# vlaxose/jstsp19

Measured on AMD Instinct MI355X. Metric: channel-estimates/sec (batched MC) at Nt=Nr=64,K=64; NMSE vs ref, higher is better.
Workload: dtype c32 (storage and results fp32 complex; big contractions as split-f16 MFMA with fp32 accumulation, fp32-equivalent); 1 GPU; proposed_algorithm approximate Imax=100, Nt=Nr=64 Nrf=8 K=64 L=8 (N=64 M=4096 Gr=64 G2=512); Imax=100, outputs=S,Y,convergence_error, pilots=per-trial (B per trial), parallelism=trials sharded, dp1

## Files before the change

include/jstsp.h:

```cpp
#ifndef JSTSP_H
#define JSTSP_H

#include <stddef.h>
#include <stdint.h>

#ifdef __cplusplus
extern "C" {
#endif

typedef struct jstsp_ctx jstsp_ctx;
typedef struct { float re, im; } jstsp_c32;
typedef struct { double re, im; } jstsp_c64;

enum { JSTSP_HOST = 0, JSTSP_DEVICE = 1 };

enum {
    JSTSP_OK = 0,
    JSTSP_E_NULL = -1,
    JSTSP_E_SHAPE = -2,
    JSTSP_E_UNSUPPORTED = -3,
    JSTSP_E_ARG = -4,
    JSTSP_E_NOMEM = -5,
    JSTSP_E_ILLCOND = -6
};

enum { JSTSP_TYPE_APPROXIMATE = 0, JSTSP_TYPE_STD = 1 };

int  jstsp_create(int device_id, jstsp_ctx **out);
int  jstsp_destroy(jstsp_ctx *ctx);
int  jstsp_set_stream(jstsp_ctx *ctx, void *hip_stream);
int  jstsp_use_own_stream(jstsp_ctx *ctx);
int  jstsp_synchronize(jstsp_ctx *ctx);
const char *jstsp_last_error(void);
const char *jstsp_version(void);
size_t jstsp_workspace_bytes(const jstsp_ctx *ctx);




int jstsp_correlate_c32(jstsp_ctx *ctx, int N, int M, int Gr, int G2, int batch,
                        const jstsp_c32 *K, const jstsp_c32 *A, long long strideA,
                        const jstsp_c32 *B, long long strideB,
                        jstsp_c32 *out, int memspace);

int jstsp_synthesize_c32(jstsp_ctx *ctx, int N, int M, int Gr, int G2, int batch,
                         const jstsp_c32 *S, const jstsp_c32 *A, long long strideA,
                         const jstsp_c32 *B, long long strideB,
                         jstsp_c32 *out, int memspace);

int jstsp_gradient_head_c32(jstsp_ctx *ctx, int N, int Gr, int G2, int batch, const jstsp_c32 *Tc,
                            const jstsp_c32 *A, long long strideA, const jstsp_c32 *GA, long long strideG,
                            const jstsp_c32 *RV, jstsp_c32 *Res_out, jstsp_c32 *P1_out, int memspace);


int jstsp_proposed_algorithm_c32(jstsp_ctx *ctx, int N, int M, int Gr, int G2, int batch,
                                 const jstsp_c32 *subY, const float *Omega,
                                 const jstsp_c32 *A, long long strideA,
                                 const jstsp_c32 *B, long long strideB,
                                 int Imax, const double *tau_Y, const double *tau_S,
                                 const double *rho, int type, const int32_t *indx_S,
                                 jstsp_c32 *S_out, jstsp_c32 *Y_out, double *ce_out,
                                 int memspace);

typedef struct jstsp_pending jstsp_pending;
int jstsp_proposed_algorithm_begin_c32(jstsp_ctx *ctx, int N, int M, int Gr, int G2, int batch,
                                       const jstsp_c32 *subY, const float *Omega,
                                       const jstsp_c32 *A, long long strideA,
                                       const jstsp_c32 *B, long long strideB,
                                       int Imax, const double *tau_Y, const double *tau_S,
                                       const double *rho, int type, const int32_t *indx_S,
                                       jstsp_c32 *S_out, jstsp_c32 *Y_out, double *ce_out,
                                       jstsp_pending **pending);
int jstsp_proposed_algorithm_end(jstsp_ctx *ctx, jstsp_pending *pending, int *fallbacks);

int jstsp_last_fused_fallbacks(jstsp_ctx *ctx, int *count);

int jstsp_last_lanczos_mismatches(jstsp_ctx *ctx, int *count);

int jstsp_lambda_max_sequence_c32(jstsp_ctx *ctx, int n, int batch, int steps, const jstsp_c32 *G, float *lam, int memspace);

int jstsp_last_dictionary_block(jstsp_ctx *ctx, int *gt);

int jstsp_ls_c32(jstsp_ctx *ctx, int N, int M, int Gr, int G2, int batch, const jstsp_c32 *Y,
                 const jstsp_c32 *A, long long strideA, const jstsp_c32 *B, long long strideB,
                 jstsp_c32 *S_out, int memspace);

int jstsp_pinv_c32(jstsp_ctx *ctx, int rows, int cols, int batch, const jstsp_c32 *A, jstsp_c32 *P, int memspace);

int jstsp_last_conditioning(jstsp_ctx *ctx, double *rcond_min, double *ns_residual_max);

int jstsp_svt_c32(jstsp_ctx *ctx, int Mr, int Mt, int batch, const jstsp_c32 *Y,
                  const double *tau, jstsp_c32 *X, int memspace);

int jstsp_omp_c32(jstsp_ctx *ctx, int measures, int size_d, int batch,
                  const jstsp_c32 *A, long long strideA, const jstsp_c32 *v, int m,
                  jstsp_c32 *x_hat, int32_t *index_out, jstsp_c32 *target_out, int memspace);

int jstsp_omp_kron_c32(jstsp_ctx *ctx, int N, int M, int Gr, int G2, int batch,
                       const jstsp_c32 *Af, long long strideA, const jstsp_c32 *Bf,
                       long long strideB, const jstsp_c32 *y, int m,
                       jstsp_c32 *x_hat, int32_t *index_out, int memspace);

int jstsp_cosamp_c32(jstsp_ctx *ctx, int measures, int size_d, int batch,
                     const jstsp_c32 *A, long long strideA, const jstsp_c32 *u, int K, int iters, double tol,
                     jstsp_c32 *x_hat, int32_t *support_out, int32_t *iters_out, double *resid_out,
                     int32_t *status_out, int memspace);
int jstsp_cosamp_kron_c32(jstsp_ctx *ctx, int N, int M, int Gr, int G2, int batch,
                          const jstsp_c32 *Af, long long strideA, const jstsp_c32 *Bf, long long strideB,
                          const jstsp_c32 *y, int K, int iters, double tol,
                          jstsp_c32 *x_hat, int32_t *support_out, int32_t *iters_out, double *resid_out,
                          int32_t *status_out, int memspace);

int jstsp_mmv_omp_c32(jstsp_ctx *ctx, int N, int Gr, int S, int batch, const jstsp_c32 *A, long long strideA,
                      const jstsp_c32 *Y, int K, int pnorm, jstsp_c32 *Z_out, int32_t *index_out,
                      int32_t *count_out, int memspace);

int jstsp_sparse_admm_c32(jstsp_ctx *ctx, int Mr, int Mt, int Gr, int Gt, int batch,
                          const jstsp_c32 *Htrue, const jstsp_c32 *OH,
                          const jstsp_c32 *Dr, const jstsp_c32 *Dt, int Imax,
                          jstsp_c32 *S_out, double *ce_out, int memspace);

int jstsp_mc_svt_c32(jstsp_ctx *ctx, int Mr, int Mt, int batch, const jstsp_c32 *OH,
                     const float *Omega, int Imax, const double *tau, const double *rho,
                     jstsp_c32 *X_out, int memspace);

int jstsp_mc_admm_c32(jstsp_ctx *ctx, int Mr, int Mt, int batch, const jstsp_c32 *Htrue,
                      const jstsp_c32 *OH, const float *Omega, int Imax, const double *tau,
                      const double *rho, jstsp_c32 *X_out, double *ce_out, int memspace);

int jstsp_vamp_c32(jstsp_ctx *ctx, int M, int N, int batch, const jstsp_c32 *y, const jstsp_c32 *A,
                   long long strideA, double sigma, double L, int nit, jstsp_c32 *x_out, int memspace);

int jstsp_vamp_kron_c32(jstsp_ctx *ctx, int Na, int Gr, int G2, int batch, const jstsp_c32 *Y,
                        const jstsp_c32 *Af, long long strideA, const jstsp_c32 *Gb, long long strideG,
                        double sigma, double L, int nit, jstsp_c32 *X_out, int memspace);

int jstsp_sparse_sca_estim_f64(jstsp_ctx *ctx, long long n, const double *rhat, double rvar, double var0, double p1, double *xhat,
                               double *xvar, int memspace);
int jstsp_cawgn_estim_out_f64(jstsp_ctx *ctx, long long n, const double *y, const double *phat, double pvar, double wvar, double *zhat,
                              double *zvar, int memspace);

int jstsp_nmse_spectral_c32(jstsp_ctx *ctx, int R, int C, int batch, const jstsp_c32 *S,
                            const jstsp_c32 *Zbar, double *nmse, int memspace);

int jstsp_rate_c32(jstsp_ctx *ctx, int R, int C, int batch, const jstsp_c32 *S, const jstsp_c32 *Zbar,
                   double noise_var, double *rate, int memspace);

typedef struct jstsp_model {
    int Nt, Nr, L;
    int T_prop;
    int Mr, Mr_e;
    int Gr, Gt;
    int clusters, rays;
    int T_hbf;
    int shared_pilots;
    double noise_var;
    int beamformer;
    int rho_rule;
    double rho_scale;
    int pilots;
} jstsp_model;
enum { JSTSP_BF_ZC = 0, JSTSP_BF_DFT = 1, JSTSP_BF_QUANTIZED = 2, JSTSP_BF_QUANTIZED4 = 3 };
enum { JSTSP_RHO_MIN6 = 0, JSTSP_RHO_MAX = 1 };
enum { JSTSP_PILOTS_QAM4 = 0, JSTSP_PILOTS_GAUSS = 1 };
// ... 156 lines not shown
```

jstsp19_amd/_lib.py:

```python
from __future__ import annotations

import ctypes as C
import os

_HERE = os.path.dirname(os.path.abspath(__file__))
LIB_PATH = os.path.join(_HERE, "csrc", "libjstsp_mi355x.so")

HOST, DEVICE = 0, 1
TYPE_APPROXIMATE, TYPE_STD = 0, 1
BF_ZC, BF_DFT, BF_QUANTIZED, BF_QUANTIZED4 = 0, 1, 2, 3
RHO_MIN6, RHO_MAX = 0, 1
PILOTS_QAM4, PILOTS_GAUSS = 0, 1

c_void_p, c_int, c_ll, c_dp, c_ip = C.c_void_p, C.c_int, C.c_longlong, C.POINTER(C.c_double), C.POINTER(C.c_int)



class Model(C.Structure):
    _fields_ = [(n, c_int) for n in ("Nt", "Nr", "L", "T_prop", "Mr", "Mr_e", "Gr", "Gt", "clusters", "rays",
                                     "T_hbf", "shared_pilots")] + [("noise_var", C.c_double), ("beamformer", c_int),
                                                                   ("rho_rule", c_int), ("rho_scale", C.c_double),
                                                                   ("pilots", c_int)]


class Trials(C.Structure):
    _fields_ = [(n, c_void_p) for n in ("subY", "Omega", "A", "B", "Zbar", "H", "indx_S")] + \
               [(n, c_dp) for n in ("tau_Y", "tau_Z", "rho")] + \
               [(n, c_void_p) for n in ("Y_hbf", "A_hbf", "B_hbf", "gains", "u_r", "u_t", "noise", "qam_idx", "pilot_sym")]


class AseDesign(C.Structure):
    _fields_ = [("kind", c_int), ("n_cols", c_int), ("pool", c_int)]


SIGNATURES = {
    "jstsp_create": (c_int, [c_int, C.POINTER(c_void_p)]),
    "jstsp_destroy": (c_int, [c_void_p]),
    "jstsp_set_stream": (c_int, [c_void_p, c_void_p]),
    "jstsp_use_own_stream": (c_int, [c_void_p]),
    "jstsp_synchronize": (c_int, [c_void_p]),
    "jstsp_last_error": (C.c_char_p, []),
    "jstsp_version": (C.c_char_p, []),
    "jstsp_workspace_bytes": (C.c_size_t, [c_void_p]),
    "jstsp_correlate_c32": (c_int, [c_void_p, c_int, c_int, c_int, c_int, c_int, c_void_p, c_void_p, c_ll,
                                    c_void_p, c_ll, c_void_p, c_int]),
    "jstsp_synthesize_c32": (c_int, [c_void_p, c_int, c_int, c_int, c_int, c_int, c_void_p, c_void_p, c_ll,
                                     c_void_p, c_ll, c_void_p, c_int]),
    "jstsp_gradient_head_c32": (c_int, [c_void_p, c_int, c_int, c_int, c_int, c_void_p, c_void_p, c_ll, c_void_p, c_ll,
                                        c_void_p, c_void_p, c_void_p, c_int]),
    "jstsp_proposed_algorithm_c32": (c_int, [c_void_p, c_int, c_int, c_int, c_int, c_int, c_void_p, c_void_p,
                                             c_void_p, c_ll, c_void_p, c_ll, c_int, c_dp, c_dp, c_dp, c_int,
                                             c_void_p, c_void_p, c_void_p, c_void_p, c_int]),
    "jstsp_proposed_algorithm_begin_c32": (c_int, [c_void_p, c_int, c_int, c_int, c_int, c_int, c_void_p, c_void_p,
                                                   c_void_p, c_ll, c_void_p, c_ll, c_int, c_dp, c_dp, c_dp, c_int,
                                                   c_void_p, c_void_p, c_void_p, c_void_p, C.POINTER(c_void_p)]),
    "jstsp_proposed_algorithm_end": (c_int, [c_void_p, c_void_p, c_ip]),
    "jstsp_ls_c32": (c_int, [c_void_p, c_int, c_int, c_int, c_int, c_int, c_void_p, c_void_p, c_ll, c_void_p, c_ll,
                             c_void_p, c_int]),
    "jstsp_pinv_c32": (c_int, [c_void_p, c_int, c_int, c_int, c_void_p, c_void_p, c_int]),
    "jstsp_last_conditioning": (c_int, [c_void_p, c_dp, c_dp]),
    "jstsp_last_fused_fallbacks": (c_int, [c_void_p, c_ip]),
    "jstsp_last_lanczos_mismatches": (c_int, [c_void_p, c_ip]),
    "jstsp_last_dictionary_block": (c_int, [c_void_p, c_ip]),
    "jstsp_svt_c32": (c_int, [c_void_p, c_int, c_int, c_int, c_void_p, c_dp, c_void_p, c_int]),
    "jstsp_omp_c32": (c_int, [c_void_p, c_int, c_int, c_int, c_void_p, c_ll, c_void_p, c_int, c_void_p,
                              c_void_p, c_void_p, c_int]),
    "jstsp_omp_kron_c32": (c_int, [c_void_p, c_int, c_int, c_int, c_int, c_int, c_void_p, c_ll, c_void_p, c_ll,
                                   c_void_p, c_int, c_void_p, c_void_p, c_int]),
    "jstsp_cosamp_c32": (c_int, [c_void_p, c_int, c_int, c_int, c_void_p, c_ll, c_void_p, c_int, c_int, C.c_double, c_void_p,
                                 c_void_p, c_void_p, c_void_p, c_void_p, c_int]),
    "jstsp_cosamp_kron_c32": (c_int, [c_void_p, c_int, c_int, c_int, c_int, c_int, c_void_p, c_ll, c_void_p, c_ll, c_void_p,
                                      c_int, c_int, C.c_double, c_void_p, c_void_p, c_void_p, c_void_p, c_void_p, c_int]),
    "jstsp_mmv_omp_c32": (c_int, [c_void_p, c_int, c_int, c_int, c_int, c_void_p, c_ll, c_void_p, c_int, c_int, c_void_p,
                                  c_void_p, c_void_p, c_int]),
    "jstsp_rate_c32": (c_int, [c_void_p, c_int, c_int, c_int, c_void_p, c_void_p, C.c_double, c_void_p, c_int]),
    "jstsp_sparse_admm_c32": (c_int, [c_void_p, c_int, c_int, c_int, c_int, c_int, c_void_p, c_void_p,
                                      c_void_p, c_void_p, c_int, c_void_p, c_void_p, c_int]),
    "jstsp_mc_svt_c32": (c_int, [c_void_p, c_int, c_int, c_int, c_void_p, c_void_p, c_int, c_dp, c_dp,
                                 c_void_p, c_int]),
    "jstsp_mc_admm_c32": (c_int, [c_void_p, c_int, c_int, c_int, c_void_p, c_void_p, c_void_p, c_int, c_dp,
                                  c_dp, c_void_p, c_void_p, c_int]),
    "jstsp_vamp_c32": (c_int, [c_void_p, c_int, c_int, c_int, c_void_p, c_void_p, c_ll, C.c_double, C.c_double, c_int,
                               c_void_p, c_int]),
    "jstsp_vamp_kron_c32": (c_int, [c_void_p, c_int, c_int, c_int, c_int, c_void_p, c_void_p, c_ll, c_void_p, c_ll,
                                    C.c_double, C.c_double, c_int, c_void_p, c_int]),
    "jstsp_sparse_sca_estim_f64": (c_int, [c_void_p, c_ll, c_void_p, C.c_double, C.c_double, C.c_double, c_void_p, c_void_p, c_int]),
    "jstsp_cawgn_estim_out_f64": (c_int, [c_void_p, c_ll, c_void_p, c_void_p, C.c_double, C.c_double, c_void_p, c_dp, c_int]),
    "jstsp_lambda_max_sequence_c32": (c_int, [c_void_p, c_int, c_int, c_int, c_void_p, c_void_p, c_int]),
    "jstsp_nmse_spectral_c32": (c_int, [c_void_p, c_int, c_int, c_int, c_void_p, c_void_p, c_void_p, c_int]),
    "jstsp_build_trials_c32": (c_int, [c_void_p, C.POINTER(Model), C.c_uint64, c_int, c_ll, c_int, C.POINTER(Trials),
                                       c_int]),
    "jstsp_beamformer_c32": (c_int, [c_void_p, c_int, c_int, c_void_p, c_int]),
    "jstsp_ase_c32": (c_int, [c_void_p, c_int, c_int, c_int, c_int, c_int, c_void_p, c_void_p, c_void_p, C.c_double, c_void_p,
                              c_int]),
    "jstsp_ase_trials_c32": (c_int, [c_void_p, C.POINTER(Model), C.POINTER(AseDesign), c_int, C.c_uint64, c_int, c_ll, c_int,
                                     c_void_p, c_void_p, c_int]),
    "jstsp_singular_values_c32": (c_int, [c_void_p, c_int, c_int, c_int, c_void_p, c_void_p, c_int]),
    "jstsp_rank_trials_c32": (c_int, [c_void_p, C.POINTER(Model), C.c_uint64, c_int, c_ll, c_int, c_int, c_void_p, c_int]),
    "jstsp_set_profiling": (c_int, [c_void_p, c_int]),
    "jstsp_get_profile": (c_int, [c_void_p, C.c_char_p, c_ip, c_dp]),
}


for _n in ("correlate", "synthesize", "proposed_algorithm", "svt", "omp", "sparse_admm", "mc_svt", "mc_admm", "vamp", "ls", "pinv",
           "mmv_omp", "vamp_kron", "nmse_spectral", "rate", "beamformer", "ase", "singular_values", "cosamp", "cosamp_kron"):
    SIGNATURES["jstsp_%s_c64" % _n] = SIGNATURES["jstsp_%s_c32" % _n]


for _n in ("correlate", "synthesize", "proposed_algorithm", "svt"):
    SIGNATURES["jstsp_%s_f64" % _n] = SIGNATURES["jstsp_%s_c32" % _n]

SIGNATURES["jstsp_pinv_f64"] = (c_int, [c_void_p, c_int, c_int, c_int, c_void_p, c_void_p, c_void_p, c_void_p, c_int])
SIGNATURES["jstsp_ls_f64"] = (c_int, [c_void_p, c_int, c_int, c_int, c_int, c_int, c_void_p, c_void_p, c_ll, c_void_p, c_ll,
                                      c_void_p, c_void_p, c_int])

SIGNATURES["jstsp_proposed_std_f64"] = (c_int, [c_void_p, c_int, c_int, c_int, c_int, c_int, c_void_p, c_void_p, c_void_p, c_ll,
                                                c_void_p, c_ll, c_void_p, c_void_p, c_int, c_dp, c_dp, c_dp, c_void_p, c_void_p,
                                                c_void_p, c_void_p, c_void_p, c_int])

for _n in ("mmv_omp", "mc_svt", "mc_admm"):
    SIGNATURES["jstsp_%s_f64" % _n] = SIGNATURES["jstsp_%s_c32" % _n]

for _n in ("omp", "omp_kron", "sparse_admm"):
    SIGNATURES["jstsp_%s_f64" % _n] = SIGNATURES["jstsp_%s_c32" % _n]


class JstspError(RuntimeError):

    def __init__(self, msg, code=None):
        super().__init__(msg)
        self.code = code


E_UNSUPPORTED, E_ILLCOND = -3, -6


_lib = None


def load():
    global _lib
    if _lib is not None:
        return _lib
    if not os.path.exists(LIB_PATH):
        raise JstspError(
            "%s is missing: build it with `python -m jstsp19_amd.build` (hipcc, gfx950). "
# ... 99 lines not shown
```

jstsp19_amd/csrc/api_misc.hip:

```cpp
#include "solver_common.h"
#include <algorithm>

namespace jstsp {

__global__ __launch_bounds__(256) void diff_kernel(long long n, const float2 *a, const float2 *b, float2 *o)
{
    const long long stride = (long long)gridDim.x * 256;
    for (long long i = (long long)blockIdx.x * 256 + threadIdx.x; i < n; i += stride)
        o[i] = make_float2(a[i].x - b[i].x, a[i].y - b[i].y);
}

__global__ void ratio_cap_kernel(int batch, const float *num, const float *den, double *out, int cap,
                                 long long ostride, long long ooff)
{
    const int t = blockIdx.x * 256 + threadIdx.x;
    if (t < batch) {
        double e = (double)num[t] / (double)den[t];
        if (cap && e > 1.0) e = 1.0;
        out[(long long)t * ostride + ooff] = e;
    }
}

__global__ __launch_bounds__(256) void mc_svt_update_kernel(long long nm, float2 *Y, const float2 *OH,
                                                            const float *Omega, const float2 *X,
// ... 580 lines not shown
    if (want_ce) need += GramWS::bytes(Mr, Mt, batch, false);
    if (memspace == JSTSP_HOST) need += 2 * rnd256(batch * nm * sizeof(float2)) + rnd256(batch * nm * sizeof(float));
    JSTSP_TRY(ctx->arena.reserve(need));
    ctx->arena.reset();
    const float2 *OH, *Htrue = nullptr;
    const float *Omega;
    JSTSP_TRY(stage_in(ctx, reinterpret_cast<const float2 *>(OH_), batch * nm, memspace, &OH));
    JSTSP_TRY(stage_in(ctx, Omega_, batch * nm, memspace, &Omega));
    if (want_ce) JSTSP_TRY(stage_in(ctx, reinterpret_cast<const float2 *>(Htrue_), batch * nm, memspace, &Htrue));
    TrialParams *prm = ctx->arena.get<TrialParams>(batch);
    float2 *X = ctx->arena.get<float2>(batch * nm), *Y = ctx->arena.get<float2>(batch * nm),
           *Z = ctx->arena.get<float2>(batch * nm), *Zn = ctx->arena.get<float2>(batch * nm),
           *D = ctx->arena.get<float2>(batch * nm);
    float *invD = ctx->arena.get<float>(batch * nm);
    float *num = ctx->arena.get<float>(batch), *den = ctx->arena.get<float>(batch);
    double *ce = ctx->arena.get<double>((size_t)batch * std::max(Imax, 1));
    JSTSP_REQUIRE(prm && X && Y && Z && Zn && D && invD && num && den && ce, JSTSP_E_NOMEM,
                  "mc_admm: workspace exhausted");
    GramWS w, wn;
    JSTSP_TRY(w.alloc(ctx->arena, Mr, Mt, batch, true));
    w.eig_stop = mc_eig_stop();
    if (want_ce) JSTSP_TRY(wn.alloc(ctx->arena, Mr, Mt, batch, false));
    JSTSP_TRY(upload_tau_rho(ctx, batch, tau, rho, prm));
    hipStream_t st = ctx->stream;
    JSTSP_HIP(hipMemsetAsync(X, 0, batch * nm * sizeof(float2), st));
    JSTSP_HIP(hipMemsetAsync(Y, 0, batch * nm * sizeof(float2), st));
    JSTSP_HIP(hipMemsetAsync(Z, 0, batch * nm * sizeof(float2), st));
    JSTSP_HIP(hipMemsetAsync(Zn, 0, batch * nm * sizeof(float2), st));
    JSTSP_TRY(launch_inv_d(ctx, (long long)nm, batch, Omega, 1.f, prm, invD));
    if (want_ce) JSTSP_TRY(sigma_max_sq(ctx, wn, Htrue, den));
    if (want_ce) JSTSP_TRY(lanczos_warm_reset(ctx, wn));
    const long long tot = (long long)batch * nm;
    for (int it = 0; it < Imax; ++it) {
        JSTSP_TRY(svt_batched(ctx, w, Zn, prm, nullptr, X, true));
        hipLaunchKernelGGL(mc_admm_update_kernel, grid2((long long)nm, batch), dim3(256), 0, st, (long long)nm,
                           Y, Z, OH, invD, X, prm, Zn);
        if (want_ce) {
            hipLaunchKernelGGL(diff_kernel, dim3((unsigned)std::min<long long>((tot + 255) / 256, 4096)),
                               dim3(256), 0, st, tot, X, Htrue, D);
            JSTSP_TRY(sigma_max_sq(ctx, wn, D, num, true));
            hipLaunchKernelGGL(ratio_cap_kernel, dim3((batch + 255) / 256), dim3(256), 0, st, batch, num, den,
                               ce, 0, (long long)Imax, (long long)it);
        }
    }
    JSTSP_HIP(hipGetLastError());
    JSTSP_TRY(stage_out(ctx, reinterpret_cast<float2 *>(X_out), X, batch * nm, memspace));
    if (want_ce && Imax > 0) JSTSP_TRY(stage_out(ctx, ce_out, ce, (size_t)batch * Imax, memspace));
    if (memspace == JSTSP_HOST) JSTSP_HIP(hipStreamSynchronize(st));
    return 0;
}

}

extern "C" int jstsp_gradient_head_c32(jstsp_ctx *ctx, int N, int Gr, int G2, int batch, const jstsp_c32 *Tc_, const jstsp_c32 *A_,
                                       long long strideA, const jstsp_c32 *GA_, long long strideG, const jstsp_c32 *RV_,
                                       jstsp_c32 *Res_out, jstsp_c32 *P1_out, int memspace)
{
    JSTSP_TRY(check_common(ctx, memspace));
    JSTSP_ENTER(ctx);
    JSTSP_REQUIRE(Tc_ && A_ && GA_ && Res_out && P1_out, JSTSP_E_NULL, "gradient_head: NULL array argument");
    JSTSP_REQUIRE(batch > 0 && grad_head_shape_ok(N, Gr, G2), JSTSP_E_UNSUPPORTED,
                  "gradient_head: N = %d, Gr = %d, G2 = %d (needs N = Gr = 64, G2 a multiple of 64)", N, Gr, G2);
    const size_t ng = (size_t)N * G2, g = (size_t)Gr * G2;
    const size_t szA = strideA ? (size_t)strideA * (batch - 1) + (size_t)N * Gr : (size_t)N * Gr;
    const size_t szG = strideG ? (size_t)strideG * (batch - 1) + (size_t)Gr * Gr : (size_t)Gr * Gr;
    size_t need = 2 * rnd256(batch * g * sizeof(float2));
    if (memspace == JSTSP_HOST)
        need += rnd256(batch * ng * sizeof(float2)) + rnd256(szA * sizeof(float2)) + rnd256(szG * sizeof(float2)) + rnd256(batch * g * sizeof(float2));
    JSTSP_TRY(ctx->arena.reserve(need));
    ctx->arena.reset();
    const float2 *Tc, *A, *GA, *RV = nullptr;
    JSTSP_TRY(stage_in(ctx, reinterpret_cast<const float2 *>(Tc_), batch * ng, memspace, &Tc));
    JSTSP_TRY(stage_in(ctx, reinterpret_cast<const float2 *>(A_), szA, memspace, &A));
    JSTSP_TRY(stage_in(ctx, reinterpret_cast<const float2 *>(GA_), szG, memspace, &GA));
    if (RV_) JSTSP_TRY(stage_in(ctx, reinterpret_cast<const float2 *>(RV_), batch * g, memspace, &RV));
    float2 *Res = ctx->arena.get<float2>(batch * g), *P1 = ctx->arena.get<float2>(batch * g);
    JSTSP_REQUIRE(Res && P1, JSTSP_E_NOMEM, "gradient_head: workspace exhausted");
    JSTSP_TRY(launch_grad_head(ctx, G2, batch, Tc, (long long)ng, 0, 1, nullptr, nullptr, 0, A, strideA, GA, strideG, RV, nullptr, Res, P1, nullptr));
    JSTSP_TRY(stage_out(ctx, reinterpret_cast<float2 *>(Res_out), Res, batch * g, memspace));
    JSTSP_TRY(stage_out(ctx, reinterpret_cast<float2 *>(P1_out), P1, batch * g, memspace));
    if (memspace == JSTSP_HOST) JSTSP_HIP(hipStreamSynchronize(ctx->stream));
    return 0;
}
```

jstsp19_amd/csrc/common.h:

```cpp
#pragma once
#include <hip/hip_runtime.h>
#include <cstdint>
#include <cstdio>
#include <cstdarg>
#include <string>
#include <vector>
#include <map>
#include "../../include/jstsp.h"

namespace jstsp {

void set_error(const char *fmt, ...);

#define JSTSP_HIP(call)                                                                  \
    do {                                                                                 \
        hipError_t e_ = (call);                                                          \
        if (e_ != hipSuccess) {                                                          \
            jstsp::set_error("%s failed: %s (%s:%d)", #call, hipGetErrorString(e_),      \
                             __FILE__, __LINE__);                                        \
            return (int)e_;                                                              \
        }                                                                                \
    } while (0)

#define JSTSP_TRY(expr)                                                                  \
// ... 152 lines not shown
    hipEvent_t pinned_done = nullptr;
    bool pinned_pending = false;
    uint32_t *diag = nullptr;
    unsigned *lz_mismatch = nullptr;
    void *hpin = nullptr;
    size_t hpin_cap = 0;
    hipEvent_t hpin_done = nullptr;
    bool hpin_pending = false;
    int dict_block_hint = 0;
    int last_dict_block = 0;
    int fused_fallbacks = 0;
    float2 *unit = nullptr;
    double2 *unit64 = nullptr;
    jstsp_ctx *helper = nullptr;
    hipStream_t side[2] = {nullptr, nullptr};
    hipStream_t cu_stream[4] = {nullptr, nullptr, nullptr, nullptr};
    int cu_state = 0;
    hipStream_t bj_stream[3] = {nullptr, nullptr, nullptr};
    hipEvent_t bj_ev[6] = {nullptr, nullptr, nullptr, nullptr, nullptr, nullptr};
    hipEvent_t ev[10] = {nullptr, nullptr, nullptr, nullptr, nullptr, nullptr, nullptr, nullptr, nullptr, nullptr};
};

namespace jstsp {

struct GemmDesc {
    const float2 *A; long long sAt, sAi, sAk; int conjA;
    const float2 *B; long long sBt, sBk, sBj; int conjB;
    const float2 *B2;
    float2 *C; long long sCt; int ldc;
    const float2 *D; long long sDt; int ldd;
    float alpha, beta;
    int m, n, k, batch;
    int splitk; long long sCsplit;
    int epi;
    const TrialParams *prm;
    float2 *e_rw0, *e_w1, *e_w2, *e_w3;
    const float2 *e_r0, *e_r1, *e_r2, *e_r3;
    const float *e_f0;
    int epi_store_c;
    uint32_t *amax_x, *amax_v1, *amax_z;
    uint32_t *amax_out;
    int force_m64;
    float2 *C_lo;
    int herm_upper;
    int sa_mode;
    const float *sa_lr, *sa_lt;
    float sa_rho, sa_thr;
};
__device__ __forceinline__ float sadmm_den(float lr, float lt, float rho) { return fmaf(lr, lt, -rho); }
__device__ __forceinline__ float sadmm_dual1(float z, float r, float s, float rho) { return fmaf(rho, r - s, z); }
__device__ __forceinline__ float sadmm_soft1(float r, float z, float ir, float thr)
{
    const float v = fmaf(ir, z, r);
    const float m = fmaxf(fabsf(v) - thr, 0.f);
    return (v > 0.f) ? m : ((v < 0.f) ? -m : 0.f);
}
__device__ __forceinline__ float sadmm_rhs1(float z, float s, float a, float rho) { return fmaf(-rho, s, z) + a; }
enum { EPI_NONE = 0, EPI_UPDATE_C = 1, EPI_UPDATE_X = 2, EPI_SADMM = 3 };
enum { GEMM_MISC = 0, GEMM_CORRELATE = 1, GEMM_SYNTH = 2, GEMM_GRAM = 3 };
int launch_cgemm(jstsp_ctx *ctx, const GemmDesc &d, int tag = GEMM_MISC);

struct HPack {
    uint4 *data = nullptr;
    uint32_t *bmax = nullptr;
    int KS = 0, JT = 0, count = 0;
    long long st = 0;
};
struct HGemmDesc {
    const float2 *A; long long sAt, sAk;
    const uint32_t *amax;
    const uint4 *Bp; long long sPt;
    const uint32_t *bmax; int sbmax;
    int KS, JT;
    float2 *C; long long sCt; int ldc;
    int m, n, k, batch;
    int epi;
    const TrialParams *prm;
    const float2 *e_r0;
    float2 *e_rw0;
    uint32_t *amax_v2;
    const uint4 *Ap; long long sApt; int aKS;
    int herm_upper;
    int map_tb, map_tt;
};
int hermitian_fill_lower(jstsp_ctx *ctx, float2 *G, long long sGt, int n, int count);
int launch_hgram(jstsp_ctx *ctx, const float2 *Z, long long sZt, int rows, int cols, int count, int nsplit,
                 const uint32_t *amax, float2 *Gpart, const float2 *Z2 = nullptr,
                 const TrialParams *zprm = nullptr,
                 bool norm_only = false);
int launch_hgram3(jstsp_ctx *ctx, const float2 *X, const float2 *V1, long long sZt, int rows, int cols, int count, int nsplit,
                  const uint32_t *xmax, const uint32_t *vmax, const uint32_t *zmax, const TrialParams *prm, float2 *Gz,
                  float2 *Gx, float2 *Gv);
size_t hgemm_pack_bytes(int Kd, int J, int count);
bool hgemm_pair_shape(int m, int n, int batch);
int hgemm_absmax(jstsp_ctx *ctx, const float2 *X, long long n, long long sXt, int count, uint32_t *amax);
int hgemm_pack(jstsp_ctx *ctx, HPack &p, Arena &ar, const float2 *B, long long sBt, long long sBk, long long sBj,
               int conj, int Kd, int J, int count, long long n_contig, const uint32_t *bmax_known = nullptr);
int hgemm_repack(jstsp_ctx *ctx, const HPack &p, const float2 *B, long long sBt, long long sBk, long long sBj, int conj,
                 int Kd, int J, const uint32_t *bmax);
int launch_hgemm(jstsp_ctx *ctx, const HGemmDesc &d, const char *prof_name = nullptr);
bool use_hgemm(long long m, long long n, long long k);

enum { EIG_SVT_Q = 0, EIG_LMAX = 1, EIG_VECS = 2 };
int launch_eig(jstsp_ctx *ctx, int mode, int n, int batch, const float2 *Gpart, long long sGt,
               int nsplit, long long sGs, const TrialParams *prm, const float *tau,
               float2 *Q, float *lam_out, float2 *Vg);
bool eig_needs_global_v(int n);
int launch_eig_large(jstsp_ctx *ctx, int mode, int n, int batch, const float2 *Gpart, long long sGt, int nsplit,
                     long long sGs, const TrialParams *prm, const float *tau, float2 *Q, float *lam_out);
int launch_eig_fast(jstsp_ctx *ctx, int mode, int n, int batch, const float2 *Gpart, long long sGt, int nsplit,
                    long long sGs, const TrialParams *prm, const float *tau, float2 *Q, float *lam_out,
                    float2 *Uwarm, int warm);
int launch_eig128(jstsp_ctx *ctx, int n, int batch, const float2 *Gpart, long long sGt, int nsplit, long long sGs,
                  const TrialParams *prm, const float *tau, float2 *Q, float2 *Uwarm = nullptr, int warm = 0,
                  int max_sweeps = 16, float stop_level = 0.f);
int eig_fast_ne(int n);
struct LanczosWarm {
    float2 *x = nullptr;
    int *state = nullptr;
    unsigned *mismatch = nullptr;
    int ne = 0;
    int call = 0;
};
int lanczos_ne(int n);
int launch_lmax(jstsp_ctx *ctx, int n, int batch, const float2 *Gpart, long long sGt, int nsplit, long long sGs,
                float *lam_out, bool lanczos = false, const LanczosWarm *lw = nullptr, int first = 0);

int launch_form_z(jstsp_ctx *ctx, long long nm, int batch, const float2 *X, const float2 *V1,
                  const TrialParams *prm, float2 *Z);
int launch_update_x(jstsp_ctx *ctx, long long nm, int batch, float2 *X, float2 *V1,
                    const float2 *V2, const float2 *C, const float2 *Xs, const float2 *Y,
                    const float2 *subY, const float *invD, const TrialParams *prm, float2 *K);
int launch_update_c(jstsp_ctx *ctx, long long nm, int batch, const float2 *X, const float2 *Xs,
                    float2 *V2, float2 *C, const TrialParams *prm);
int launch_step_v(jstsp_ctx *ctx, int g, int batch, const float2 *Res, const float2 *RRes,
                  float2 *V, float2 *S, const int32_t *rank, int cnt, const TrialParams *prm,
                  double *ce3, int Imax, int it, float2 *RV = nullptr, int waves8 = 0,
                  uint32_t *zero8 = nullptr);
int launch_soft(jstsp_ctx *ctx, int g, int batch, const float2 *V, float2 *S, const int32_t *rank,
                int cnt, const TrialParams *prm);
int launch_inv_d(jstsp_ctx *ctx, long long nm, int batch, const float *Omega, float scale2rho,
                 const TrialParams *prm, float *invD);
int launch_rank_from_index(jstsp_ctx *ctx, int g, int batch, const int32_t *indx, int32_t *rank);
int launch_eye_minus(jstsp_ctx *ctx, int n, int count, const float2 *Q, float2 *P);
int launch_ce_ratio(jstsp_ctx *ctx, int batch, const float *lamV1, const float *lamV2,
                    const float *lamX, double *ce, int Imax, int it);

void prof_begin(jstsp_ctx *ctx, const char *name);
void prof_end(jstsp_ctx *ctx, const char *name);

}
```

jstsp19_amd/csrc/fused.hip:

```cpp
#include "solver_common.h"
#include <algorithm>
#include <cstdlib>
#include <cstdio>

namespace jstsp {
namespace {

typedef _Float16 half8 __attribute__((ext_vector_type(8)));
typedef _Float16 half4 __attribute__((ext_vector_type(4)));
typedef float f32x4 __attribute__((ext_vector_type(4)));

constexpr int FPAD = 128;

__device__ __host__ inline int fscale_exp(uint32_t amax_bits)
{
    const int be = (int)((amax_bits >> 23) & 0xff);
    if (be == 0 || be == 255) return 0;
    return 13 - (be - 127);
}
__device__ __forceinline__ void fsplit(float x, _Float16 &h, _Float16 &l)
{
    h = (_Float16)x;
    l = (_Float16)(x - (float)h);
}
typedef unsigned int u32x4 __attribute__((ext_vector_type(4)));
typedef unsigned int u32x2 __attribute__((ext_vector_type(2)));
__device__ __forceinline__ u32x4 negu(u32x4 u) { return u ^ 0x80008000u; }
template <class T> __device__ __forceinline__ T ldg(const void *base, uint32_t boff)
{
    return *reinterpret_cast<const T *>(reinterpret_cast<const char *>(base) + boff);
}
template <class T> __device__ __forceinline__ T ldg_nt(const void *base, uint32_t boff)
{
    return __builtin_nontemporal_load(reinterpret_cast<const T *>(reinterpret_cast<const char *>(base) + boff));
}
typedef float f32x2 __attribute__((ext_vector_type(2)));
__device__ __forceinline__ float2 ldg_nt2(const void *base, uint32_t boff)
{
    const f32x2 v = ldg_nt<f32x2>(base, boff);
    return make_float2(v.x, v.y);
}
__device__ __forceinline__ void stg_nt2(void *base, uint32_t boff, float2 v)
{
    __builtin_nontemporal_store(f32x2{v.x, v.y}, reinterpret_cast<f32x2 *>(reinterpret_cast<char *>(base) + boff));
}
template <class T> __device__ __forceinline__ void stg(void *base, uint32_t boff, T v)
{
    *reinterpret_cast<T *>(reinterpret_cast<char *>(base) + boff) = v;
}
__device__ __forceinline__ f32x4 mma(u32x4 a, u32x4 b, f32x4 c)
{
    return __builtin_amdgcn_mfma_f32_16x16x32_f16(__builtin_bit_cast(half8, a), __builtin_bit_cast(half8, b), c, 0, 0, 0);
}

__global__ __launch_bounds__(256) void pack_bf_kernel(const float2 *B, long long sBt, int G2, int M, const uint32_t *bmax,
                                                      int sbmax, uint4 *out, long long sOut)
{
    const int t = blockIdx.y;
    const int G8 = G2 >> 3;
    const long long per_tile = 32ll * G8;
    const long long idx = (long long)blockIdx.x * 256 + threadIdx.x;
    if (idx >= (long long)(M / 32) * per_tile) return;
    const int tile = (int)(idx / per_tile);
    int rem = (int)(idx % per_tile);
    const int g8 = rem % G8; rem /= G8;
    const int r = rem & 3, mq = rem >> 2;
    const int m = tile * 32 + 4 * mq + r;
    const float s = ldexpf(1.f, fscale_exp(bmax[(long long)t * sbmax]));
    half8 pl[4];
#pragma unroll
    for (int c = 0; c < 8; ++c) {
        const float2 x = B[(long long)t * sBt + (8 * g8 + c) + (long long)G2 * m];
        _Float16 h, l;
        fsplit(x.x * s, h, l); pl[0][c] = h; pl[1][c] = l;
        fsplit(x.y * s, h, l); pl[2][c] = h; pl[3][c] = l;
    }
    uint4 *o = out + (long long)t * sOut + (long long)tile * (16ll * G2);
    const int blk = g8 >> 1, g8i = g8 & 1;
#pragma unroll
    for (int p = 0; p < 4; ++p) o[(((long long)(blk * 4 + p) * 8 + mq) * 2 + g8i) * 4 + r] = *reinterpret_cast<uint4 *>(&pl[p]);
}

__global__ __launch_bounds__(256) void toeplitz_probe_kernel(const float2 *B, long long sBt, int G2, int M, uint32_t cand, uint32_t *mism)
{
    const uint32_t idx = blockIdx.x * 256u + threadIdx.x;
    uint32_t bad = 0;
    if (idx < (uint32_t)G2 * (uint32_t)M) {
        const int m = (int)(idx / (uint32_t)G2), g = (int)(idx - (uint32_t)m * (uint32_t)G2);
        const uint2 *b = reinterpret_cast<const uint2 *>(B) + (long long)blockIdx.y * sBt;
        const uint2 x = b[idx];
#pragma unroll
        for (int c = 0; c < 5; ++c) {
            const int gt = 16 << c, ld = g >> (4 + c);
            if (!((cand >> c) & 1u) || ld == 0 || m < ld) continue;
            const uint2 y = b[idx - (uint32_t)gt - (uint32_t)G2];
            if (x.x != y.x || x.y != y.y) bad |= 1u << c;
        }
    }
#pragma unroll
    for (int o = 32; o > 0; o >>= 1) bad |= __shfl_xor(bad, o);
    if ((threadIdx.x & 63) == 0 && (bad & ~__atomic_load_n(mism, __ATOMIC_RELAXED))) atomicOr(mism, bad);
}

__global__ __launch_bounds__(256) void toeplitz_verify_kernel(const float2 *B, long long sBt, int G2, int M, int c, uint32_t *mism)
{
    const uint32_t q = blockIdx.x * 256u + threadIdx.x;
    const uint32_t qpc = (uint32_t)G2 >> 2;
    uint32_t bad = 0;
    if (q < qpc * (uint32_t)M) {
        const int m = (int)(q / qpc), g = 4 * (int)(q - (uint32_t)m * qpc);
        const int gt = 16 << c, ld = g >> (4 + c);
        if (ld >= 1 && m >= ld) {
            const uint4 *b = reinterpret_cast<const uint4 *>(reinterpret_cast<const uint2 *>(B) + (long long)blockIdx.y * sBt);
            const uint32_t e = (uint32_t)g + (uint32_t)G2 * (uint32_t)m;
            const uint4 x0 = b[e >> 1], x1 = b[(e >> 1) + 1];
            const uint32_t f = e - (uint32_t)gt - (uint32_t)G2;
            const uint4 y0 = b[f >> 1], y1 = b[(f >> 1) + 1];
            if (x0.x != y0.x || x0.y != y0.y || x0.z != y0.z || x0.w != y0.w || x1.x != y1.x || x1.y != y1.y || x1.z != y1.z ||
                x1.w != y1.w)
                bad = 1u << c;
        }
    }
#pragma unroll
    for (int o = 32; o > 0; o >>= 1) bad |= __shfl_xor(bad, o);
    if ((threadIdx.x & 63) == 0 && (bad & ~__atomic_load_n(mism, __ATOMIC_RELAXED))) atomicOr(mism, bad);
}

__global__ __launch_bounds__(256) void pack_e_kernel(const float2 *B, long long sBt, int G2, int M, int gt, int ecols, int ehalo,
                                                     const uint32_t *bmax, int sbmax, uint4 *out, long long sOut)
{
    const int t = blockIdx.y;
    const int G8t = gt >> 3, L = G2 / gt;
    const long long idx = (long long)blockIdx.x * 256 + threadIdx.x;
    if (idx >= (long long)G8t * ecols) return;
    const int g8 = (int)(idx % G8t), j = (int)(idx / G8t);
    int row0 = 8 * g8, m = j - ehalo;
    bool live = true;
    if (m < 0) {
        const int jh = -m;
        int ld = 1;
        while (ld * (ld + 1) / 2 < jh) ++ld;
        live = ld < L;
        const int c = -(jh - ld * (ld - 1) / 2);
        m = c + ld; row0 += ld * gt;
    }
    const float s = ldexpf(1.f, fscale_exp(bmax[(long long)t * sbmax]));
    half8 pl[4];
#pragma unroll
    for (int c = 0; c < 8; ++c) {
        const float2 x = live ? B[(long long)t * sBt + (row0 + c) + (long long)G2 * m] : make_float2(0.f, 0.f);
        _Float16 h, l;
        fsplit(x.x * s, h, l); pl[0][c] = h; pl[1][c] = l;
        fsplit(x.y * s, h, l); pl[2][c] = h; pl[3][c] = l;
    }
    uint4 *o = out + (long long)t * sOut;
#pragma unroll
    for (int p = 0; p < 4; ++p) o[(long long)(p * G8t + g8) * ecols + j] = *reinterpret_cast<uint4 *>(&pl[p]);
}

__host__ __device__ inline int eswz(int x) { return (((x >> 1) & 3) << 1) | ((x >> 3) & 1); }

__global__ __launch_bounds__(256) void pack_e2_kernel(const float2 *B, long long sBt, int G2, int M, const uint32_t *bmax, int sbmax,
                                                      uint4 *out, long long sOut, float2 *Bdl)
{
    const int t = blockIdx.y;
    const int idx = blockIdx.x * 256 + threadIdx.x;
    if (idx < G2 * 8)
        Bdl[(long long)t * G2 * 8 + idx] = B[(long long)t * sBt + (idx >> 3) + (long long)G2 * (idx & 7)];
    if (idx >= (M + 8) * 8) return;
    const int o = idx & 7, cc = idx >> 3, m = cc - 7;
    const bool live = m >= 0 && m < M;
    const float s = ldexpf(1.f, fscale_exp(bmax[(long long)t * sbmax]));
    half8 pl[4];
#pragma unroll
    for (int c = 0; c < 8; ++c) {
        const float2 x = live ? B[(long long)t * sBt + (8 * o + c) + (long long)G2 * m] : make_float2(0.f, 0.f);
        _Float16 h, l;
        fsplit(x.x * s, h, l); pl[0][c] = h; pl[1][c] = l;
        fsplit(x.y * s, h, l); pl[2][c] = h; pl[3][c] = l;
    }
    uint4 *dst = out + (long long)t * sOut;
#pragma unroll
    for (int p = 0; p < 4; ++p) dst[((long long)p * (M + 8) + cc) * 8 + (o ^ eswz(cc))] = *reinterpret_cast<uint4 *>(&pl[p]);
}

__device__ __forceinline__ void xs_delta(const float2 *W, const float2 *Bdl, int G2, int m, int r, float2 *out)
{
    __shared__ float2 part[4][64];
    const int lane = threadIdx.x & 63, wv = threadIdx.x >> 6;
    const int g0 = 64 * (m + 1), cnt = G2 - g0;
    float2 a = make_float2(0.f, 0.f), a2 = a;
    const int per = (cnt + 15) / 16, lo = min(g0 + (4 * r + wv) * per, G2), hi = min(lo + per, G2);
    int g = lo;
    for (; g + 8 <= hi; g += 8) {
        float2 w[8], b[8];
#pragma unroll
        for (int u = 0; u < 8; ++u) { w[u] = W[lane + 64ll * (g + u)]; b[u] = Bdl[(g + u) * 8 + m]; }
#pragma unroll
        for (int u = 0; u < 8; u += 2) {
            a.x = fmaf(w[u].x, b[u].x, fmaf(-w[u].y, b[u].y, a.x)); a.y = fmaf(w[u].x, b[u].y, fmaf(w[u].y, b[u].x, a.y));
            a2.x = fmaf(w[u + 1].x, b[u + 1].x, fmaf(-w[u + 1].y, b[u + 1].y, a2.x));
            a2.y = fmaf(w[u + 1].x, b[u + 1].y, fmaf(w[u + 1].y, b[u + 1].x, a2.y));
        }
    }
    for (; g < hi; ++g) {
        const float2 w0 = W[lane + 64ll * g], b0 = Bdl[g * 8 + m];
        a.x = fmaf(w0.x, b0.x, fmaf(-w0.y, b0.y, a.x)); a.y = fmaf(w0.x, b0.y, fmaf(w0.y, b0.x, a.y));
    }
// ... 676 lines not shown
                const u32x4 k2 = *reinterpret_cast<const u32x4 *>(kp + 2048), k3 = *reinterpret_cast<const u32x4 *>(kp + 3072);
                f32x4 tr = mma(bf[0], k0, f32x4{0.f, 0.f, 0.f, 0.f}), ti = mma(bf[0], k2, f32x4{0.f, 0.f, 0.f, 0.f});
                tr = mma(bf[0], k1, tr); ti = mma(bf[0], k3, ti);
                tr = mma(bf[1], k0, tr); ti = mma(bf[1], k2, ti);
                k0 = *reinterpret_cast<const u32x4 *>(kp + 4096); k1 = *reinterpret_cast<const u32x4 *>(kp + 5120);
                tr = mma(bf[2], k2, tr); ti = mma(bf[2], k0, ti);
                tr = mma(bf[2], k3, tr); ti = mma(bf[2], k1, ti);
                tr = mma(bf[3], k2, tr); ti = mma(bf[3], k0, ti);
                {
                    const int grp = 4 * gb + n2;
                    if (grp >= 6 && grp - 6 < 12) F64_STORE(grp - 6, (i + 1) & 1, rf[((grp - 6) >> 2) & 1][(grp - 6) & 3])
                    if (grp < 12) F64_LOAD(grp, tn, rf[(grp >> 2) & 1][grp & 3])
                }
                pr[gb][n2] += tr; pi[gb][n2] += ti;
                __builtin_amdgcn_sched_barrier(0);
            }
        }
        {
            constexpr int NG = 4 * GB;
#pragma unroll
            for (int pc = (NG > 6 ? NG - 6 : 0); pc < 12; ++pc) {
                if (pc >= NG) F64_LOAD(pc, tn, rf[(pc >> 2) & 1][pc & 3])
                F64_STORE(pc, (i + 1) & 1, rf[(pc >> 2) & 1][pc & 3])
            }
        }
        __builtin_amdgcn_sched_barrier(0);
        F64_WQLOAD()
        __syncthreads();
    }
#undef F64_LOAD
#undef F64_STORE
#undef F64_FLD
#undef F64_J
#undef F64_WQLOAD
    float2 *po = d.Ppart + ((long long)t * d.parts + part) * (64ll * G2);
#pragma unroll
    for (int gb = 0; gb < GB; ++gb)
#pragma unroll
        for (int n2 = 0; n2 < 4; ++n2)
#pragma unroll
            for (int s = 0; s < 4; ++s) {
                const int g = 16 * GB * w + 16 * gb + 4 * q + s;
                po[64ll * g + 16 * n2 + c16] = make_float2(pr[gb][n2][s] * sp, pi[gb][n2][s] * sp);
            }
#pragma unroll
    for (int o = 32; o > 0; o >>= 1) {
        kmx = fmaxf(kmx, __shfl_xor(kmx, o)); xmx = fmaxf(xmx, __shfl_xor(xmx, o)); v1mx = fmaxf(v1mx, __shfl_xor(v1mx, o));
        zmx = fmaxf(zmx, __shfl_xor(zmx, o)); v2mx = fmaxf(v2mx, __shfl_xor(v2mx, o));
    }
    if (l == 0) {
        if (d.kmax_out) atomicMax(&d.kmax_out[t], __float_as_uint(kmx));
        if (d.xmax) atomicMax(&d.xmax[t], __float_as_uint(xmx));
        if (d.v1max) atomicMax(&d.v1max[t], __float_as_uint(v1mx));
        if (d.zmax) atomicMax(&d.zmax[t], __float_as_uint(zmx));
        if (d.v2max) atomicMax(&d.v2max[t], __float_as_uint(v2mx));
        if (d.ovf && !(kmx * sk < 60000.f)) atomicOr(&d.ovf[t], 1u);
    }
}

}

bool fused_shape_ok(int N, int M, int G2, int parts)
{
    return N == 64 && G2 >= 128 && G2 <= 512 && G2 % 128 == 0 && parts > 0 && M % (32 * parts) == 0;
}

static void compact_dims(int M, int G2, int gt, int *ecols, int *ehalo)
{
    const int L = G2 / gt;
    *ehalo = ((L * (L - 1) / 2 + 3) / 4) * 4;
    *ecols = *ehalo + M;
}

size_t fused_bytes(int M, int G2, int nB, int batch, int parts)
{
    int ec, eh;
    compact_dims(M, G2, 16, &ec, &eh);
    return rnd256((size_t)nB * (M / 32) * 16 * G2 * sizeof(uint4)) + rnd256((size_t)batch * (G2 / 32) * 1024 * sizeof(uint4)) +
           rnd256((size_t)batch * parts * 64 * G2 * sizeof(float2)) + rnd256((size_t)batch * sizeof(uint32_t)) + rnd256((size_t)batch * 2048 * sizeof(uint4)) +
           rnd256((size_t)nB * 4 * (G2 / 16) * ec * sizeof(uint4)) + 5 * rnd256((size_t)batch * 512 * sizeof(float2)) +
           rnd256((size_t)nB * G2 * 8 * sizeof(float2)) + 512;
}

int fused_probe_toeplitz(jstsp_ctx *ctx, Arena &ar, const float2 *B, long long sBt, int G2, int M, int nB, int *gt)
{
    *gt = 0;
    uint32_t *flag = ar.get<uint32_t>(1);
    JSTSP_REQUIRE(flag, JSTSP_E_NOMEM, "fused pass: workspace exhausted");
    JSTSP_REQUIRE((long long)G2 * M < (1ll << 31), JSTSP_E_UNSUPPORTED, "fused pass: dictionary too large");
    uint32_t cand = 0;
    for (int c = 0; c < 5; ++c)
        if (G2 % (16 << c) == 0 && 2 * (16 << c) <= G2) cand |= 1u << c;
    const unsigned nblk = (unsigned)(((long long)G2 * M + 255) / 256);
    for (int step = 0; step < (nB > 1 ? 2 : 1) && cand; ++step) {
        JSTSP_HIP(hipMemsetAsync(flag, 0, sizeof(uint32_t), ctx->stream));
        if (step && sBt % 2 == 0)
            hipLaunchKernelGGL(toeplitz_verify_kernel, dim3((nblk + 3) / 4, nB), dim3(256), 0, ctx->stream, B, sBt, G2, M,
                               31 - __builtin_clz(cand), flag);
        else
            hipLaunchKernelGGL(toeplitz_probe_kernel, dim3(nblk, step ? nB : 1), dim3(256), 0, ctx->stream, B, sBt, G2, M, cand, flag);
        JSTSP_HIP(hipGetLastError());
        uint32_t bad = ~0u;
        JSTSP_HIP(hipMemcpyAsync(&bad, flag, sizeof(uint32_t), hipMemcpyDeviceToHost, ctx->stream));
        JSTSP_HIP(hipStreamSynchronize(ctx->stream));
        cand &= ~bad;
        cand &= cand ? (~cand + 1u) : 0u;
    }
    if (cand) *gt = 16 << (31 - __builtin_clz(cand));
    return 0;
}

__global__ __launch_bounds__(256) void toeplitz_gram_kernel(const float2 *B, long long sBt, int G2, int M, int gt, const float2 *G0,
                                                            const float2 *G0lo, float2 *G, float2 *Glo)
{
    const int t = blockIdx.y;
    const int idx = blockIdx.x * 256 + threadIdx.x;
    if (idx >= G2 * G2) return;
    const int r = idx % G2, c = idx / G2;
    const int ld = r / gt, g = r - ld * gt, l2 = c / gt, g2 = c - l2 * gt;
    if (ld > l2) return;
    const int d = l2 - ld;
    const float2 *b = B + (long long)t * sBt;
    const long long i0 = (long long)t * gt * G2 + g + (long long)gt * (d * gt + g2);
    double vr = (double)G0[i0].x + (G0lo ? (double)G0lo[i0].x : 0.0), vi = (double)G0[i0].y + (G0lo ? (double)G0lo[i0].y : 0.0);
    auto mac = [&](float2 x, float2 y, double sgn) {
        vr += sgn * ((double)x.x * y.x + (double)x.y * y.y);
        vi += sgn * ((double)x.y * y.x - (double)x.x * y.y);
    };
    for (int m = 0; m < d; ++m) mac(b[g + (long long)G2 * m], b[d * gt + g2 + (long long)G2 * m], -1.0);
    for (int u = M - ld; u < M; ++u) mac(b[g + (long long)G2 * u], b[g2 + (long long)G2 * (u - d)], -1.0);
    for (int m = 0; m < l2; ++m) mac(b[r + (long long)G2 * m], b[c + (long long)G2 * m], 1.0);
    if (r == c) vi = 0.0;
    const float hr = (float)vr, hi = (float)vi;
    float2 *o = G + (long long)t * G2 * G2;
    o[r + (long long)G2 * c] = make_float2(hr, hi);
    if (ld < l2) o[c + (long long)G2 * r] = make_float2(hr, -hi);
    if (Glo) {
        float2 *ol = Glo + (long long)t * G2 * G2;
        const float lr = (float)(vr - (double)hr), li = (float)(vi - (double)hi);
        ol[r + (long long)G2 * c] = make_float2(lr, li);
        if (ld < l2) ol[c + (long long)G2 * r] = make_float2(lr, -li);
    }
}

int toeplitz_gram_assemble(jstsp_ctx *ctx, const float2 *B, long long sBt, int G2, int M, int gt, int nB, const float2 *G0,
                           const float2 *G0lo, float2 *G, float2 *Glo)
{
    hipLaunchKernelGGL(toeplitz_gram_kernel, dim3((unsigned)((G2 * G2 + 255) / 256), nB), dim3(256), 0, ctx->stream, B, sBt, G2, M, gt,
                       G0, G0lo, G, Glo);
    JSTSP_HIP(hipGetLastError());
    return 0;
}

int fused_alloc(Arena &ar, FusedWS &f, int M, int G2, int nB, int batch, int parts, int gt, int v2)
{
    f.parts = parts;
    f.sBf = (long long)(M / 32) * 16 * G2;
    f.sAS = (long long)(G2 / 32) * 1024;
    f.gt = gt;
    f.v2 = (gt == 64 && v2) ? 1 : 0;
    if (f.v2) {
        f.ecols = M + 8; f.ehalo = 7;
        f.sEc = 4ll * f.ecols * 8;
        f.Ec = ar.get<uint4>((size_t)nB * f.sEc);
        f.XsD = ar.get<float2>((size_t)batch * 2048);
        f.Kf = ar.get<float2>((size_t)batch * 512);
        f.Bdl = ar.get<float2>((size_t)nB * G2 * 8);
        JSTSP_REQUIRE(f.XsD && f.Kf && f.Bdl, JSTSP_E_NOMEM, "fused pass: workspace exhausted");
    } else if (gt) {
        compact_dims(M, G2, gt, &f.ecols, &f.ehalo);
        f.sEc = 4ll * (gt / 8) * f.ecols;
        f.Ec = ar.get<uint4>((size_t)nB * f.sEc);
    } else
        f.Bf = ar.get<uint4>((size_t)nB * f.sBf);
    f.ASp = ar.get<uint4>((size_t)batch * f.sAS);
    f.Ppart = ar.get<float2>((size_t)batch * parts * 64 * G2);
    f.ovf = ar.get<uint32_t>(batch);
    f.Wqp = ar.get<uint4>((size_t)batch * 2048);
    JSTSP_REQUIRE((f.Bf || f.Ec) && f.ASp && f.Ppart && f.ovf && f.Wqp, JSTSP_E_NOMEM, "fused pass: workspace exhausted");
    return 0;
}

int fused_pack_b(jstsp_ctx *ctx, FusedWS &f, const float2 *B, long long sBt, int G2, int M, int nB, const uint32_t *bmax)
// ... 105 lines not shown
```

jstsp19_amd/csrc/hgemm.hip:

```cpp
#include "solver_common.h"
#include <type_traits>

namespace jstsp {

typedef _Float16 half8 __attribute__((ext_vector_type(8)));
typedef float f32x16 __attribute__((ext_vector_type(16)));
typedef unsigned int u32x4 __attribute__((ext_vector_type(4)));

namespace {

constexpr int HBK = 32;
constexpr int FLUSH = 8;
constexpr float LO_SCALE = 1.f, LO_INV = 1.f;

__device__ __host__ inline int scale_exp(uint32_t amax_bits)
{
    const int be = (int)((amax_bits >> 23) & 0xff);
    if (be == 0 || be == 255) return 0;
    return 13 - (be - 127);
}

__device__ __forceinline__ void split2(float x, _Float16 &h, _Float16 &l)
{
    h = (_Float16)x;
    l = (_Float16)((x - (float)h) * LO_SCALE);
}

__global__ __launch_bounds__(256) void absmax_kernel(long long n2, const float *X, long long sXt, uint32_t *amax)
{
    const int t = blockIdx.y;
    const float *p = X + (long long)t * sXt;
    float m = 0.f;
    const bool vec = ((sXt & 3) == 0) && ((n2 & 3) == 0) && (((uintptr_t)X & 15) == 0);
    if (vec) {
        const float4 *p4 = reinterpret_cast<const float4 *>(p);
        for (long long i = (long long)blockIdx.x * 256 + threadIdx.x; i < n2 / 4; i += (long long)gridDim.x * 256) {
            const float4 v = p4[i];
            m = fmaxf(fmaxf(m, fmaxf(fabsf(v.x), fabsf(v.y))), fmaxf(fabsf(v.z), fabsf(v.w)));
        }
    } else {
        for (long long i = (long long)blockIdx.x * 256 + threadIdx.x; i < n2; i += (long long)gridDim.x * 256)
            m = fmaxf(m, fabsf(p[i]));
    }
    for (int o = 32; o > 0; o >>= 1) m = fmaxf(m, __shfl_xor(m, o));
    __shared__ float sm[4];
    if ((threadIdx.x & 63) == 0) sm[threadIdx.x >> 6] = m;
    __syncthreads();
    if (threadIdx.x == 0)
        atomicMax(&amax[t], __float_as_uint(fmaxf(fmaxf(sm[0], sm[1]), fmaxf(sm[2], sm[3]))));
}

__global__ __launch_bounds__(256) void pack_b_kernel(const float2 *B, long long sBt, long long sBk, long long sBj,
                                                     int conj, int Kd, int J, int KS, int JT, const uint32_t *bmax,
                                                     uint4 *out)
{
    const int t = blockIdx.y;
    const long long idx = (long long)blockIdx.x * 256 + threadIdx.x;
    if (idx >= (long long)JT * KS * 64) return;
    const int lane = (int)(idx & 63);
    const long long blk = idx >> 6;
    const int ks = (int)(blk % KS), jt = (int)(blk / KS);
    const int j = jt * 32 + (lane & 31), k0 = ks * 16 + 8 * (lane >> 5);
    const float s = ldexpf(1.f, scale_exp(bmax[t]));
    const float sg = conj ? -s : s;
    half8 rh, rl, ih, il;
#pragma unroll
    for (int v = 0; v < 8; ++v) {
        float2 x = make_float2(0.f, 0.f);
        if (j < J && k0 + v < Kd) x = B[(long long)t * sBt + (long long)(k0 + v) * sBk + (long long)j * sBj];
        _Float16 h, l;
        split2(x.x * s, h, l); rh[v] = h; rl[v] = l;
        split2(x.y * sg, h, l); ih[v] = h; il[v] = l;
    }
    uint4 *o = out + (((long long)t * JT + jt) * KS + ks) * 256 + lane;
    o[0] = *reinterpret_cast<uint4 *>(&rh);
    o[64] = *reinterpret_cast<uint4 *>(&rl);
    o[128] = *reinterpret_cast<uint4 *>(&ih);
    o[192] = *reinterpret_cast<uint4 *>(&il);
}

__device__ __forceinline__ half8 as_half8(uint4 u) { return *reinterpret_cast<half8 *>(&u); }
__device__ __forceinline__ half8 neg_half8(uint4 u)
{
    u.x ^= 0x80008000u; u.y ^= 0x80008000u; u.z ^= 0x80008000u; u.w ^= 0x80008000u;
    return *reinterpret_cast<half8 *>(&u);
}

__device__ __forceinline__ bool block_to_trial_tile(const HGemmDesc &d, int tiles, int &t, int &tile)
{
    const int bid = blockIdx.x;
    const int xcd = bid & 7, slot = bid >> 3;
    if (d.map_tb == 0) {
        t = (slot / tiles) * 8 + xcd;
        tile = slot % tiles;
        return t < d.batch;
    }
    const int per = d.map_tb * d.map_tt;
    const int nbt = (d.batch + d.map_tb - 1) / d.map_tb;
    const int blk = (slot / per) * 8 + xcd, w = slot % per;
    t = (blk % nbt) * d.map_tb + w % d.map_tb;
    tile = (blk / nbt) * d.map_tt + w / d.map_tb;
    return t < d.batch && tile < tiles;
}

template <int EPI, bool APACK, int WJ, bool EVEN = false>
__global__ __launch_bounds__(128 * WJ, WJ == 2 ? 2 : 2) void hgemm_kernel(HGemmDesc d, int tiles_i, int tiles_j)
{
    constexpr int STG = 1024 + 512 * WJ;
    constexpr int NA = (WJ == 2) ? 8 : 4;
    __shared__ uint4 smem[2 * STG];

    const int tiles = tiles_i * tiles_j;
    int t, rem;
    if (!block_to_trial_tile(d, tiles, t, rem)) return;
    const int ti = rem % tiles_i, tj = rem / tiles_i;
    const int i0 = ti * 64, j0 = tj * 32 * WJ;
    if (d.herm_upper && i0 >= j0 + 32 * WJ) return;

    const int tid = threadIdx.x, lane = tid & 63, wave = tid >> 6;
    const int wi = wave & 1, wj = wave >> 1;

    const int ea = scale_exp(d.amax[t]);
    const int eb = scale_exp(d.bmax[(long long)t * d.sbmax]);
    const float sa = ldexpf(1.f, ea);

    const int ai = tid & 63, akg = tid >> 6;
    const bool arow = (i0 + ai) < d.m;
    const float2 *abase = APACK ? nullptr : d.A + (long long)t * d.sAt;
    const float2 *pa = APACK ? nullptr : abase + (arow ? (i0 + ai) : 0) + (long long)(NA * akg) * d.sAk;
    const int a_slot = (WJ == 2) ? ((((ai >> 5) * 2 + (akg >> 1)) * 4) * 64) + (akg & 1) * 32 + (ai & 31)
                                 : ((((ai >> 5) * 2 + (akg >> 2)) * 4) * 64) + ((akg >> 1) & 1) * 32 + (ai & 31);
    const uint4 *pb = d.Bp + (long long)t * d.sPt + ((long long)(tj * WJ) * d.KS) * 256 + lane;
    const int nst = d.KS / 2;
    const int kfull = d.k / HBK;

    struct StgF { float2 a[NA]; uint4 b0, b1, b2, b3; };
    struct StgP { u32x4 a0, a1, a2, a3; uint4 b0, b1, b2, b3; };
    using Stg = typename std::conditional<APACK, StgP, StgF>::type;
    const uint4 *pbw = pb + ((long long)(wave >> 1) * d.KS + (wave & 1)) * 256;
    const uint4 *paw = APACK ? d.Ap + (long long)t * d.sApt + lane +
                                   ((long long)(ti * 2 + (wave >> 1)) * d.KS + (wave & 1)) * 256
                             : nullptr;
    const float sa_m = arow ? sa : 0.f;
    auto load = [&](int s_in, Stg &R) {
        const int s = EVEN ? (s_in < nst ? s_in : 0) : s_in;
        const uint4 *g = pbw + (long long)(2 * s) * 256;
        const u32x4 *gn = reinterpret_cast<const u32x4 *>(g);
        const u32x4 x0 = __builtin_nontemporal_load(gn), x1 = __builtin_nontemporal_load(gn + 64),
                    x2 = __builtin_nontemporal_load(gn + 128), x3 = __builtin_nontemporal_load(gn + 192);
        R.b0 = make_uint4(x0.x, x0.y, x0.z, x0.w); R.b1 = make_uint4(x1.x, x1.y, x1.z, x1.w);
        R.b2 = make_uint4(x2.x, x2.y, x2.z, x2.w); R.b3 = make_uint4(x3.x, x3.y, x3.z, x3.w);
        if constexpr (APACK) {
            const u32x4 *ga = reinterpret_cast<const u32x4 *>(paw + (long long)(2 * s) * 256);
            R.a0 = ga[0]; R.a1 = ga[64]; R.a2 = ga[128]; R.a3 = ga[192];
        } else {
            if (EVEN || s < kfull) {
#pragma unroll
                for (int v = 0; v < NA; ++v) R.a[v] = pa[(long long)(s * HBK + v) * d.sAk];
            } else {
                const int kbase = s * HBK + NA * akg;
#pragma unroll
                for (int v = 0; v < NA; ++v) {
                    const bool ok = kbase + v < d.k;
                    const float2 *p = ok ? pa + (long long)(s * HBK + v) * d.sAk : abase;
                    const float2 x = *p;
                    R.a[v] = ok ? x : make_float2(0.f, 0.f);
                }
            }
        }
    };
    auto store = [&](const Stg &R, uint4 *buf) {
        uint4 *o = buf + 1024 + wave * 256 + lane;
        o[0] = R.b0; o[64] = R.b1; o[128] = R.b2; o[192] = R.b3;
        if constexpr (APACK) {
            u32x4 *q = reinterpret_cast<u32x4 *>(buf + wave * 256 + lane);
            q[0] = R.a0; q[64] = R.a1; q[128] = R.a2; q[192] = R.a3;
        } else {
            half8 rh = {0}, rl = {0}, ih = {0}, il = {0};
#pragma unroll
            for (int v = 0; v < NA; ++v) {
                _Float16 h, l;
                split2(R.a[v].x * sa_m, h, l); rh[v] = h; rl[v] = l;
                split2(R.a[v].y * sa_m, h, l); ih[v] = h; il[v] = l;
            }
            if constexpr (WJ == 2) {
                uint4 *q = buf + a_slot;
                q[0] = *reinterpret_cast<uint4 *>(&rh);
                q[64] = *reinterpret_cast<uint4 *>(&rl);
                q[128] = *reinterpret_cast<uint4 *>(&ih);
                q[192] = *reinterpret_cast<uint4 *>(&il);
            } else {
                uint2 *q = reinterpret_cast<uint2 *>(buf + a_slot) + (akg & 1);
                q[0] = *reinterpret_cast<uint2 *>(&rh);
                q[2 * 64] = *reinterpret_cast<uint2 *>(&rl);
                q[2 * 128] = *reinterpret_cast<uint2 *>(&ih);
                q[2 * 192] = *reinterpret_cast<uint2 *>(&il);
            }
        }
    };

    f32x16 re_h = {0}, re_l = {0}, im_h = {0}, im_l = {0};
    f32x16 Lre = {0}, Lim = {0};
    auto fold = [&]() {
#pragma unroll
        for (int r = 0; r < 16; ++r) {
            Lre[r] += re_h[r] + re_l[r] * LO_INV;
            Lim[r] += im_h[r] + im_l[r] * LO_INV;
            re_h[r] = 0.f; re_l[r] = 0.f; im_h[r] = 0.f; im_l[r] = 0.f;
        }
    };
    auto compute = [&](const uint4 *buf) {
#pragma unroll
        for (int ks = 0; ks < 2; ++ks) {
            const uint4 *fa = buf + ((wi * 2 + ks) * 4) * 64 + lane;
            const uint4 *fb = buf + 1024 + ((wj * 2 + ks) * 4) * 64 + lane;
            const uint4 uar_h = fa[0], uar_l = fa[64], uai_h = fa[128], uai_l = fa[192];
            const half8 br_h = as_half8(fb[0]), br_l = as_half8(fb[64]), bi_h = as_half8(fb[128]), bi_l = as_half8(fb[192]);
            const half8 ar_h = as_half8(uar_h), ar_l = as_half8(uar_l), ai_h = as_half8(uai_h), ai_l = as_half8(uai_l);
            const half8 nai_h = neg_half8(uai_h), nai_l = neg_half8(uai_l);
            re_h = __builtin_amdgcn_mfma_f32_32x32x16_f16(br_h, ar_h, re_h, 0, 0, 0);
            re_l = __builtin_amdgcn_mfma_f32_32x32x16_f16(br_l, ar_h, re_l, 0, 0, 0);
            im_h = __builtin_amdgcn_mfma_f32_32x32x16_f16(bi_h, ar_h, im_h, 0, 0, 0);
            im_l = __builtin_amdgcn_mfma_f32_32x32x16_f16(bi_l, ar_h, im_l, 0, 0, 0);
            re_h = __builtin_amdgcn_mfma_f32_32x32x16_f16(bi_h, nai_h, re_h, 0, 0, 0);
            re_l = __builtin_amdgcn_mfma_f32_32x32x16_f16(br_h, ar_l, re_l, 0, 0, 0);
            im_h = __builtin_amdgcn_mfma_f32_32x32x16_f16(br_h, ai_h, im_h, 0, 0, 0);
            im_l = __builtin_amdgcn_mfma_f32_32x32x16_f16(bi_h, ar_l, im_l, 0, 0, 0);
            re_l = __builtin_amdgcn_mfma_f32_32x32x16_f16(bi_l, nai_h, re_l, 0, 0, 0);
            im_l = __builtin_amdgcn_mfma_f32_32x32x16_f16(br_l, ai_h, im_l, 0, 0, 0);
            re_l = __builtin_amdgcn_mfma_f32_32x32x16_f16(bi_h, nai_l, re_l, 0, 0, 0);
            im_l = __builtin_amdgcn_mfma_f32_32x32x16_f16(br_h, ai_l, im_l, 0, 0, 0);
        }
    };
    auto stage = [&](int s, const uint4 *cur, uint4 *nxt, Stg &Rnear, Stg &Rfar) {
        if (EVEN || s + 2 < nst) load(s + 2, Rfar);
        compute(cur);
        asm volatile("" ::: "memory");
        __builtin_amdgcn_sched_barrier(0);
        if (EVEN || s + 1 < nst) store(Rnear, nxt);
        if (((s + 1) % FLUSH) == 0) fold();
        __syncthreads();
    };

    Stg R0, R1;
    uint4 *buf0 = smem, *buf1 = smem + STG;
    load(0, R0);
    if (EVEN || nst > 1) load(1, R1);
    store(R0, buf0);
    __syncthreads();

    for (int s = 0; s < nst; s += 2) {
        stage(s, buf0, buf1, R1, R0);
        if (EVEN || s + 1 < nst) stage(s + 1, buf1, buf0, R0, R1);
    }
    fold();

// ... 35 lines not shown
    const bool vec4 = ((d.m & 1) == 0) && ((d.ldc & 1) == 0) && ((d.sCt & 1) == 0) && (((uintptr_t)d.C & 15) == 0) &&
                      (EPI != EPI_UPDATE_C || ((((uintptr_t)d.e_r0 | (uintptr_t)d.e_rw0) & 15) == 0));
    const TrialParams prm = (EPI == EPI_UPDATE_C) ? d.prm[t] : TrialParams();
    auto swap1 = [](float x) {
        return __builtin_bit_cast(float, __builtin_amdgcn_update_dpp(0, __builtin_bit_cast(int, x), 0xB1, 0xf, 0xf, false));
    };
    if (vec4) {
        const bool odd = lane & 1;
#pragma unroll
        for (int it = 0; it < 2; ++it) {
            const int gi = it * 32 + (lane & 31);
            const int gi2 = gi & ~1;
            float4 xs[8];
            long long ixs[8];
            bool ok[8];
#pragma unroll
            for (int rp = 0; rp < 8; ++rp) {
                const int r0 = 2 * rp, r1 = r0 + 1;
                const float2 o0 = make_float2(re[it][r0] * alpha, im[it][r0] * alpha);
                const float2 o1 = make_float2(re[it][r1] * alpha, im[it][r1] * alpha);
                const float2 snd = odd ? o0 : o1;
                const float2 rcv = make_float2(swap1(snd.x), swap1(snd.y));
                xs[rp] = odd ? make_float4(rcv.x, rcv.y, o1.x, o1.y) : make_float4(o0.x, o0.y, rcv.x, rcv.y);
                const int gj = jw0 + (r0 & 3) + 8 * (r0 >> 2) + 4 * (lane >> 5) + (odd ? 1 : 0);
                ok[rp] = gi2 < d.m && gj < d.n;
                ixs[rp] = (long long)t * d.sCt + (ok[rp] ? gi2 + (long long)gj * d.ldc : 0);
            }
            if (EPI == EPI_UPDATE_C) {
                float4 x[8], v2[8];
#pragma unroll
                for (int rp = 0; rp < 8; ++rp) {
                    x[rp] = *reinterpret_cast<const float4 *>(d.e_r0 + ixs[rp]);
                    v2[rp] = *reinterpret_cast<const float4 *>(d.e_rw0 + ixs[rp]);
                }
                asm volatile("" ::: "memory");
#pragma unroll
                for (int rp = 0; rp < 8; ++rp) {
                    float4 v = v2[rp];
                    v.x = admm_v2(prm, v.x, x[rp].x, xs[rp].x);
                    v.y = admm_v2(prm, v.y, x[rp].y, xs[rp].y);
                    v.z = admm_v2(prm, v.z, x[rp].z, xs[rp].z);
                    v.w = admm_v2(prm, v.w, x[rp].w, xs[rp].w);
                    if (ok[rp]) {
                        *reinterpret_cast<float4 *>(d.e_rw0 + ixs[rp]) = v;
                        vmax = fmaxf(fmaxf(vmax, fmaxf(fabsf(v.x), fabsf(v.y))), fmaxf(fabsf(v.z), fabsf(v.w)));
                    }
                }
            }
#pragma unroll
            for (int rp = 0; rp < 8; ++rp)
                if (ok[rp]) *reinterpret_cast<float4 *>(d.C + ixs[rp]) = xs[rp];
        }
    } else {
#pragma unroll
        for (int it = 0; it < 2; ++it) {
            const int gi = it * 32 + (lane & 31);
            if (gi >= d.m) continue;
#pragma unroll
            for (int r = 0; r < 16; ++r) {
                const int gj = jw0 + (r & 3) + 8 * (r >> 2) + 4 * (lane >> 5);
                if (gj >= d.n) continue;
                const float vr = re[it][r], vi = im[it][r];
                const float2 o = make_float2(vr * alpha, vi * alpha);
                const long long ix = (long long)t * d.sCt + gi + (long long)gj * d.ldc;
                if (EPI == EPI_UPDATE_C) {
                    const float2 x = d.e_r0[ix];
                    float2 v2 = d.e_rw0[ix];
                    v2.x = admm_v2(prm, v2.x, x.x, o.x);
                    v2.y = admm_v2(prm, v2.y, x.y, o.y);
                    d.e_rw0[ix] = v2;
                    vmax = fmaxf(vmax, fmaxf(fabsf(v2.x), fabsf(v2.y)));
                }
                Cp[gi + (long long)gj * d.ldc] = o;
            }
        }
    }
    if (EPI == EPI_UPDATE_C && d.amax_v2) {
#pragma unroll
        for (int o = 32; o > 0; o >>= 1) vmax = fmaxf(vmax, __shfl_xor(vmax, o));
        if (lane == 0) atomicMax(&d.amax_v2[t], __float_as_uint(vmax));
    }
}

template <int EPI, bool APACK, int NW, int PD>
__global__ __launch_bounds__(64 * NW, NW == 4 ? 2 : 1) void hgemm2_kernel(HGemmDesc d, int tiles_j)
{
    constexpr int NT = 64 * NW;
    constexpr int NA = 2048 / NT;
    constexpr int NAB = 16 / NW;
    __shared__ uint4 smem[2 * 1024];

    int t, tj;
    if (!block_to_trial_tile(d, tiles_j, t, tj)) return;
    const int j0 = tj * 32 * NW;
    const int tid = threadIdx.x, lane = tid & 63, wave = tid >> 6;

    const int ea = scale_exp(d.amax[t]);
    const int eb = scale_exp(d.bmax[(long long)t * d.sbmax]);
    const float sa = ldexpf(1.f, ea);

    const int ai = tid & 63, akg = tid >> 6;
    const bool arow = ai < d.m;
    const float2 *abase = APACK ? nullptr : d.A + (long long)t * d.sAt;
    const float2 *arow_base = APACK ? nullptr : abase + (arow ? ai : 0);
    const int a_slot = (NA == 8) ? ((((ai >> 5) * 2 + (akg >> 1)) * 4) * 64) + (akg & 1) * 32 + (ai & 31)
                                 : ((((ai >> 5) * 2 + (akg >> 2)) * 4) * 64) + ((akg >> 1) & 1) * 32 + (ai & 31);
    const float sa_m = arow ? sa : 0.f;
    const int nst = d.KS / 2;
    const uint4 *paw = nullptr;
    if constexpr (APACK) {
        const int q0 = wave * NAB;
        paw = d.Ap + (long long)t * d.sApt + lane + ((long long)(q0 >> 3) * d.KS + ((q0 >> 2) & 1)) * 256 + (q0 & 3) * 64;
    }
    struct AF { float2 a[NA]; };
    struct AP { u32x4 q[NAB]; };
    using AStg = typename std::conditional<APACK, AP, AF>::type;
    auto load_a = [&](int s, AStg &R) {
        if constexpr (APACK) {
            const u32x4 *g = reinterpret_cast<const u32x4 *>(paw + (long long)(2 * s) * 256);
#pragma unroll
            for (int r = 0; r < NAB; ++r) R.q[r] = g[r * 64];
        } else {
            const int kbase = s * HBK + NA * akg;
#pragma unroll
            for (int v = 0; v < NA; ++v) {
                const int kk = min(kbase + v, d.k - 1);
                float2 x = arow_base[(long long)kk * d.sAk];
                if (kbase + v >= d.k) x = make_float2(0.f, 0.f);
                R.a[v] = x;
            }
        }
    };
    auto store_a = [&](const AStg &R, uint4 *buf) {
        if constexpr (APACK) {
            u32x4 *q = reinterpret_cast<u32x4 *>(buf + wave * NAB * 64 + lane);
#pragma unroll
            for (int r = 0; r < NAB; ++r) q[r * 64] = R.q[r];
        } else {
            half8 rh = {0}, rl = {0}, ih = {0}, il = {0};
#pragma unroll
            for (int v = 0; v < NA; ++v) {
                _Float16 h, l;
                split2(R.a[v].x * sa_m, h, l); rh[v] = h; rl[v] = l;
                split2(R.a[v].y * sa_m, h, l); ih[v] = h; il[v] = l;
            }
            if constexpr (NA == 8) {
                uint4 *q = buf + a_slot;
                q[0] = *reinterpret_cast<uint4 *>(&rh);
                q[64] = *reinterpret_cast<uint4 *>(&rl);
                q[128] = *reinterpret_cast<uint4 *>(&ih);
                q[192] = *reinterpret_cast<uint4 *>(&il);
            } else {
                uint2 *q = reinterpret_cast<uint2 *>(buf + a_slot) + (akg & 1);
                q[0] = *reinterpret_cast<uint2 *>(&rh);
                q[2 * 64] = *reinterpret_cast<uint2 *>(&rl);
                q[2 * 128] = *reinterpret_cast<uint2 *>(&ih);
                q[2 * 192] = *reinterpret_cast<uint2 *>(&il);
            }
        }
    };

    const uint4 *pbw = d.Bp + (long long)t * d.sPt + ((long long)(tj * NW + wave) * d.KS) * 256 + lane;
    struct BStg { u32x4 q[8]; };
    const uint4 *pdummy = APACK ? d.Ap + (long long)t * d.sApt + lane : pbw;
    auto load_b_half = [&](int s, int ks, BStg &R) {
        const u32x4 *g = reinterpret_cast<const u32x4 *>(s < nst ? pbw + (long long)(2 * s + ks) * 256 : pdummy);
#pragma unroll
        for (int p = 0; p < 4; ++p) R.q[ks * 4 + p] = __builtin_nontemporal_load(g + p * 64);
    };

    f32x16 re[2], im[2];
#pragma unroll
    for (int it = 0; it < 2; ++it)
#pragma unroll
        for (int r = 0; r < 16; ++r) { re[it][r] = 0.f; im[it][r] = 0.f; }
    auto h8 = [](u32x4 u) { return *reinterpret_cast<half8 *>(&u); };
    auto nh8 = [](u32x4 u) { u.x ^= 0x80008000u; u.y ^= 0x80008000u; u.z ^= 0x80008000u; u.w ^= 0x80008000u;
                             return *reinterpret_cast<half8 *>(&u); };
    auto compute_half = [&](const uint4 *buf, int ks, const BStg &R) {
        const half8 br_h = h8(R.q[ks * 4 + 0]), br_l = h8(R.q[ks * 4 + 1]), bi_h = h8(R.q[ks * 4 + 2]),
                    bi_l = h8(R.q[ks * 4 + 3]);
        const u32x4 *fa0 = reinterpret_cast<const u32x4 *>(buf + ((0 * 2 + ks) * 4) * 64 + lane);
        const u32x4 *fa1 = reinterpret_cast<const u32x4 *>(buf + ((1 * 2 + ks) * 4) * 64 + lane);
        const u32x4 u0r_h = fa0[0], u0r_l = fa0[64], u0i_h = fa0[128], u0i_l = fa0[192];
        const u32x4 u1r_h = fa1[0], u1r_l = fa1[64], u1i_h = fa1[128], u1i_l = fa1[192];
        const half8 a0r_h = h8(u0r_h), a0r_l = h8(u0r_l), a0i_h = h8(u0i_h), a0i_l = h8(u0i_l);
        const half8 a1r_h = h8(u1r_h), a1r_l = h8(u1r_l), a1i_h = h8(u1i_h), a1i_l = h8(u1i_l);
        const half8 n0i_h = nh8(u0i_h), n0i_l = nh8(u0i_l), n1i_h = nh8(u1i_h), n1i_l = nh8(u1i_l);
        re[0] = __builtin_amdgcn_mfma_f32_32x32x16_f16(br_h, a0r_h, re[0], 0, 0, 0);
        im[0] = __builtin_amdgcn_mfma_f32_32x32x16_f16(bi_h, a0r_h, im[0], 0, 0, 0);
        re[1] = __builtin_amdgcn_mfma_f32_32x32x16_f16(br_h, a1r_h, re[1], 0, 0, 0);
        im[1] = __builtin_amdgcn_mfma_f32_32x32x16_f16(bi_h, a1r_h, im[1], 0, 0, 0);
        re[0] = __builtin_amdgcn_mfma_f32_32x32x16_f16(bi_h, n0i_h, re[0], 0, 0, 0);
        im[0] = __builtin_amdgcn_mfma_f32_32x32x16_f16(br_h, a0i_h, im[0], 0, 0, 0);
        re[1] = __builtin_amdgcn_mfma_f32_32x32x16_f16(bi_h, n1i_h, re[1], 0, 0, 0);
        im[1] = __builtin_amdgcn_mfma_f32_32x32x16_f16(br_h, a1i_h, im[1], 0, 0, 0);
        re[0] = __builtin_amdgcn_mfma_f32_32x32x16_f16(br_l, a0r_h, re[0], 0, 0, 0);
        im[0] = __builtin_amdgcn_mfma_f32_32x32x16_f16(bi_l, a0r_h, im[0], 0, 0, 0);
        re[1] = __builtin_amdgcn_mfma_f32_32x32x16_f16(br_l, a1r_h, re[1], 0, 0, 0);
        im[1] = __builtin_amdgcn_mfma_f32_32x32x16_f16(bi_l, a1r_h, im[1], 0, 0, 0);
        re[0] = __builtin_amdgcn_mfma_f32_32x32x16_f16(br_h, a0r_l, re[0], 0, 0, 0);
        im[0] = __builtin_amdgcn_mfma_f32_32x32x16_f16(bi_h, a0r_l, im[0], 0, 0, 0);
        re[1] = __builtin_amdgcn_mfma_f32_32x32x16_f16(br_h, a1r_l, re[1], 0, 0, 0);
        im[1] = __builtin_amdgcn_mfma_f32_32x32x16_f16(bi_h, a1r_l, im[1], 0, 0, 0);
        re[0] = __builtin_amdgcn_mfma_f32_32x32x16_f16(bi_l, n0i_h, re[0], 0, 0, 0);
        im[0] = __builtin_amdgcn_mfma_f32_32x32x16_f16(br_l, a0i_h, im[0], 0, 0, 0);
        re[1] = __builtin_amdgcn_mfma_f32_32x32x16_f16(bi_l, n1i_h, re[1], 0, 0, 0);
        im[1] = __builtin_amdgcn_mfma_f32_32x32x16_f16(br_l, a1i_h, im[1], 0, 0, 0);
        re[0] = __builtin_amdgcn_mfma_f32_32x32x16_f16(bi_h, n0i_l, re[0], 0, 0, 0);
        im[0] = __builtin_amdgcn_mfma_f32_32x32x16_f16(br_h, a0i_l, im[0], 0, 0, 0);
        re[1] = __builtin_amdgcn_mfma_f32_32x32x16_f16(bi_h, n1i_l, re[1], 0, 0, 0);
        im[1] = __builtin_amdgcn_mfma_f32_32x32x16_f16(br_h, a1i_l, im[1], 0, 0, 0);
    };
    const float alpha = ldexpf(1.f, -(ea + eb));
    auto stage = [&](int s, BStg &R, AStg &RAnext) {
        const uint4 *cur = smem + (s & 1) * 1024;
        const int sb = s + PD, sa2 = min(s + 1 + PD, nst - 1);
        compute_half(cur, 0, R);
        load_b_half(sb, 0, R);
        compute_half(cur, 1, R);
        load_b_half(sb, 1, R);
        asm volatile("" ::: "memory");
        __builtin_amdgcn_sched_barrier(0);
        store_a(RAnext, smem + ((s + 1) & 1) * 1024);
        load_a(sa2, RAnext);
        __syncthreads();
    };

    BStg RB[PD];
    AStg RAr[PD];
    AStg RA0;
    load_a(0, RA0);
#pragma unroll
    for (int p = 0; p < PD; ++p) {
        load_b_half(min(p, nst - 1), 0, RB[p]); load_b_half(min(p, nst - 1), 1, RB[p]);
        load_a(min(p + 1, nst - 1), RAr[p]);
    }
    store_a(RA0, smem);
    __syncthreads();
    for (int s = 0; s < nst; s += PD) {
#pragma unroll
        for (int p = 0; p < PD; ++p) stage(s + p, RB[p], RAr[p]);
    }

    rows64_epilogue<EPI>(d, t, j0 + wave * 32, re, im, alpha, lane);
}

constexpr int FLUSH2 = 16;
template <int EPI, bool TWOLVL>
__global__ __launch_bounds__(256, 1) void hgemm_pair_kernel(HGemmDesc d, int tiles_j, int npairs)
{
    constexpr int PD = 2;
    extern __shared__ uint4 smem[];

    const int bid = blockIdx.x, xcd = bid & 7, slot = bid >> 3;
    const int per = d.map_tb * d.map_tt, nbt = (npairs + d.map_tb - 1) / d.map_tb;
    const int blk = (slot / per) * 8 + xcd, wq = slot % per;
    const int tp = (blk % nbt) * d.map_tb + wq % d.map_tb;
    const int tj = (blk / nbt) * d.map_tt + wq / d.map_tb;
    if (tp >= npairs || tj >= tiles_j) return;
    const int tr0 = 2 * tp, tr1 = min(2 * tp + 1, d.batch - 1);
    const bool two = 2 * tp + 1 < d.batch;
    const int j0 = tj * 128;
    const int tid = threadIdx.x, lane = tid & 63, wave = tid >> 6;
// ... 547 lines not shown
    prof_begin(ctx, "gram");
    JSTSP_REQUIRE(!Z2 || zprm, JSTSP_E_NULL, "hgram: Z2 without per-problem scalars");
    if (norm_only && !Z2 && cols >= GRAM_HONLY_MIN_COLS) {
        if (cols % (nsplit * 2 * HBK) == 0)
            hgram_kernel<true, true><<<(unsigned)grid, 256, 0, ctx->stream>>>(Z, sZt, rows, cols, nsplit, amax, Gpart, count, Z2, zprm);
        else
            hgram_kernel<false, true><<<(unsigned)grid, 256, 0, ctx->stream>>>(Z, sZt, rows, cols, nsplit, amax, Gpart, count, Z2, zprm);
    } else
    if (cols % (nsplit * 2 * HBK) == 0)
        hgram_kernel<true><<<(unsigned)grid, 256, 0, ctx->stream>>>(Z, sZt, rows, cols, nsplit, amax, Gpart, count, Z2, zprm);
    else
        hgram_kernel<false><<<(unsigned)grid, 256, 0, ctx->stream>>>(Z, sZt, rows, cols, nsplit, amax, Gpart, count, Z2, zprm);
    prof_end(ctx, "gram");
    JSTSP_HIP(hipGetLastError());
    return 0;
}

int launch_hgram3(jstsp_ctx *ctx, const float2 *X, const float2 *V1, long long sZt, int rows, int cols, int count, int nsplit,
                  const uint32_t *xmax, const uint32_t *vmax, const uint32_t *zmax, const TrialParams *prm, float2 *Gz,
                  float2 *Gx, float2 *Gv)
{
    JSTSP_REQUIRE(rows > 0 && rows <= 64 && cols > 0 && count > 0 && nsplit > 0, JSTSP_E_SHAPE, "hgram3: bad shape");
    const long long grid = (long long)count * nsplit;
    JSTSP_REQUIRE(grid < (1ll << 31), JSTSP_E_UNSUPPORTED, "hgram3 grid too large");
    prof_begin(ctx, "gram");
    const bool nh = cols >= GRAM_HONLY_MIN_COLS;
    if (cols % (nsplit * 2 * HBK) == 0) {
        if (nh) hgram3_kernel<true, true><<<(unsigned)grid, 256, 0, ctx->stream>>>(X, V1, sZt, rows, cols, nsplit, xmax, vmax, zmax, prm, Gz, Gx, Gv, count);
        else hgram3_kernel<true, false><<<(unsigned)grid, 256, 0, ctx->stream>>>(X, V1, sZt, rows, cols, nsplit, xmax, vmax, zmax, prm, Gz, Gx, Gv, count);
    } else {
        if (nh) hgram3_kernel<false, true><<<(unsigned)grid, 256, 0, ctx->stream>>>(X, V1, sZt, rows, cols, nsplit, xmax, vmax, zmax, prm, Gz, Gx, Gv, count);
        else hgram3_kernel<false, false><<<(unsigned)grid, 256, 0, ctx->stream>>>(X, V1, sZt, rows, cols, nsplit, xmax, vmax, zmax, prm, Gz, Gx, Gv, count);
    }
    prof_end(ctx, "gram");
    JSTSP_HIP(hipGetLastError());
    return 0;
}

__global__ __launch_bounds__(256) void herm_fill_kernel(float2 *G, long long sGt, int n)
{
    __shared__ float2 tl[32][33];
    const int nt = (n + 31) / 32;
    const int bi = blockIdx.x % nt, bj = blockIdx.x / nt;
    if (bi < bj) return;
    float2 *g = G + (long long)blockIdx.y * sGt;
    const int tx = threadIdx.x & 31, ty = threadIdx.x >> 5;
    for (int y = ty; y < 32; y += 8) {
        const int r = 32 * bj + tx, c = 32 * bi + y;
        tl[y][tx] = (r < n && c < n) ? g[r + (long long)n * c] : make_float2(0.f, 0.f);
    }
    __syncthreads();
    for (int y = ty; y < 32; y += 8) {
        const int r = 32 * bi + tx, c = 32 * bj + y;
        if (r < n && c < n && r > c) g[r + (long long)n * c] = make_float2(tl[tx][y].x, -tl[tx][y].y);
    }
}

int hermitian_fill_lower(jstsp_ctx *ctx, float2 *G, long long sGt, int n, int count)
{
    const int nt = (n + 31) / 32;
    herm_fill_kernel<<<dim3((unsigned)(nt * nt), count), 256, 0, ctx->stream>>>(G, sGt, n);
    JSTSP_HIP(hipGetLastError());
    return 0;
}

static long long hgemm_grid(HGemmDesc &d, long long tiles, int conc)
{
    d.map_tb = d.map_tt = 0;
    if (d.sPt == 0 && d.batch >= 2 && tiles >= 2) {
        d.map_tb = d.batch < 8 ? d.batch : 8;
        d.map_tt = conc / d.map_tb < 1 ? 1 : conc / d.map_tb;
        if (d.map_tt > tiles) d.map_tt = (int)tiles;
        const long long nb = (long long)((d.batch + d.map_tb - 1) / d.map_tb) * ((tiles + d.map_tt - 1) / d.map_tt);
        return ((nb + 7) / 8) * 8 * d.map_tb * d.map_tt;
    }
    return (long long)((d.batch + 7) / 8) * 8 * tiles;
}

bool hgemm_pair_shape(int m, int n, int batch)
{
    return m == 64 && batch >= 2 && (long long)((batch + 1) / 2) * ((n + 127) / 128) >= 256;
}

int launch_hgemm(jstsp_ctx *ctx, const HGemmDesc &d_in, const char *prof_name)
{
    HGemmDesc d = d_in;
    JSTSP_REQUIRE(d.m > 0 && d.n > 0 && d.k > 0 && d.batch > 0, JSTSP_E_SHAPE, "hgemm: bad shape");
    JSTSP_REQUIRE(d.KS >= 2 * ((d.k + 31) / 32) && d.JT >= 2 * ((d.n + 63) / 64), JSTSP_E_ARG,
                  "hgemm: packed operand smaller than the product");
    const bool wide = !d.Ap && d.epi == EPI_NONE && d.n >= 128 && d.JT * 32 >= ((d.n + 127) / 128) * 128;
    const int tiles_i = (d.m + 63) / 64, tiles_j = wide ? (d.n + 127) / 128 : (d.n + 63) / 64;
    const bool wide_even = wide && (d.k % 32) == 0 && ((d.KS / 2) % 2) == 0 && d.KS == 2 * (d.k / 32);
    JSTSP_REQUIRE((long long)((d.batch + 7) / 8) * 8 * tiles_i * tiles_j < (1ll << 30), JSTSP_E_UNSUPPORTED, "hgemm grid too large");
    if (d.Ap && d.aKS == d.KS && d.sPt == 0 && d.sbmax == 0 && !d.herm_upper && (d.KS % 4) == 0 &&
        hgemm_pair_shape(d.m, d.n, d.batch) && d.JT * 32 >= ((d.n + 127) / 128) * 128) {
        const int npairs = (d.batch + 1) / 2, tj3 = (d.n + 127) / 128;
        d.map_tb = npairs < 4 ? npairs : 4;
        d.map_tt = 32 / d.map_tb < tj3 ? 32 / d.map_tb : tj3;
        const long long nb = (long long)((npairs + d.map_tb - 1) / d.map_tb) * ((tj3 + d.map_tt - 1) / d.map_tt);
        const long long grid3 = ((nb + 7) / 8) * 8 * d.map_tb * d.map_tt;
        JSTSP_REQUIRE(grid3 < (1ll << 31), JSTSP_E_UNSUPPORTED, "hgemm grid too large");
        if (prof_name) prof_begin(ctx, prof_name);
        constexpr int PAIR_LDS = 3 * 2048 * (int)sizeof(uint4);
        auto go = [&](auto kern, int lds) -> int {
            JSTSP_HIP(hipFuncSetAttribute(reinterpret_cast<const void *>(kern), hipFuncAttributeMaxDynamicSharedMemorySize, lds));
            hipLaunchKernelGGL(kern, dim3((unsigned)grid3), dim3(256), lds, ctx->stream, d, tj3, npairs);
            return 0;
        };
        if (d.epi == EPI_UPDATE_C) JSTSP_TRY(go(hgemm_pair_kernel<EPI_UPDATE_C, false>, PAIR_LDS));
        else if (d.k > 1024) JSTSP_TRY(go(hgemm_pair_kernel<EPI_NONE, true>, PAIR_LDS + 65536));
        else JSTSP_TRY(go(hgemm_pair_kernel<EPI_NONE, false>, PAIR_LDS));
        if (prof_name) prof_end(ctx, prof_name);
        JSTSP_HIP(hipGetLastError());
        return 0;
    }
    const int v2_mask = 1;
    const bool pack_ok = d.JT * 32 >= ((d.n + 127) / 128) * 128;
    if (d.m <= 64 && pack_ok && d.Ap && (v2_mask & 1) && d.aKS == d.KS && (d.KS % 4) == 0) {
        const int tj2 = (d.n + 127) / 128;
        const long long grid2 = hgemm_grid(d, tj2, 64);
        if (prof_name) prof_begin(ctx, prof_name);
        if (d.epi == EPI_UPDATE_C)
            hgemm2_kernel<EPI_UPDATE_C, true, 4, 2><<<(unsigned)grid2, 256, 0, ctx->stream>>>(d, tj2);
        else
            hgemm2_kernel<EPI_NONE, true, 4, 2><<<(unsigned)grid2, 256, 0, ctx->stream>>>(d, tj2);
        if (prof_name) prof_end(ctx, prof_name);
        JSTSP_HIP(hipGetLastError());
        return 0;
    }
    if (d.m <= 64 && pack_ok && !d.Ap && (v2_mask & 2) && (d.KS % 4) == 0 && d.epi == EPI_NONE && d.k <= 1024) {
        const int tj2 = (d.n + 127) / 128;
        const long long grid2 = hgemm_grid(d, tj2, 64);
        if (prof_name) prof_begin(ctx, prof_name);
        hgemm2_kernel<EPI_NONE, false, 4, 2><<<(unsigned)grid2, 256, 0, ctx->stream>>>(d, tj2);
        if (prof_name) prof_end(ctx, prof_name);
        JSTSP_HIP(hipGetLastError());
        return 0;
    }
    const long long grid = hgemm_grid(d, (long long)tiles_i * tiles_j, wide ? 32 : 64);
    if (prof_name) prof_begin(ctx, prof_name);
    if (wide_even) {
        hgemm_kernel<EPI_NONE, false, 4, true><<<(unsigned)grid, 512, 0, ctx->stream>>>(d, tiles_i, tiles_j);
    } else if (wide) {
        hgemm_kernel<EPI_NONE, false, 4><<<(unsigned)grid, 512, 0, ctx->stream>>>(d, tiles_i, tiles_j);
    } else if (d.Ap) {
        JSTSP_REQUIRE(d.aKS == d.KS, JSTSP_E_ARG, "hgemm: packed a and b operands disagree on the k padding");
        if (d.epi == EPI_UPDATE_C)
            hgemm_kernel<EPI_UPDATE_C, true, 2><<<(unsigned)grid, 256, 0, ctx->stream>>>(d, tiles_i, tiles_j);
        else
            hgemm_kernel<EPI_NONE, true, 2><<<(unsigned)grid, 256, 0, ctx->stream>>>(d, tiles_i, tiles_j);
    } else if (d.epi == EPI_UPDATE_C)
        hgemm_kernel<EPI_UPDATE_C, false, 2><<<(unsigned)grid, 256, 0, ctx->stream>>>(d, tiles_i, tiles_j);
    else
        hgemm_kernel<EPI_NONE, false, 2><<<(unsigned)grid, 256, 0, ctx->stream>>>(d, tiles_i, tiles_j);
    if (prof_name) prof_end(ctx, prof_name);
    JSTSP_HIP(hipGetLastError());
    return 0;
}

}
```

jstsp19_amd/csrc/proposed.hip:

```cpp
#include "solver_common.h"
#include <cstdio>
#include <cmath>
#include <cstdlib>
#include <algorithm>

namespace jstsp {

struct ProposedWS {
    float2 *X, *V1, *V2, *C, *Xs, *Y, *ZK, *Zb, *Zb2;
    float *invD;
    float2 *V, *RV, *Res, *RRes, *S, *P1;
    float2 *Tc, *W;
    float2 *GA, *GB;
    TrialParams *prm;
    int32_t *rank;
    double *ce;
    float *lam;
    GramWS gz, gn;
    bool h2 = false;
    HPack Bc, Bs;
    uint32_t *kmax = nullptr, *wmax = nullptr;
    uint32_t *nmax = nullptr, *zmax = nullptr;
    bool h2g = false;
    HPack GBp;
// ... 64 lines not shown
    if (want_ce) JSTSP_TRY(w.gn.alloc(a, N, M, 3 * batch, false, ns3));
    w.h2 = use_hgemm(N, G2, M);
    if (w.h2) {
        w.kmax = a.get<uint32_t>(16 * (size_t)batch);
        JSTSP_REQUIRE(w.kmax, JSTSP_E_NOMEM, "proposed_algorithm: workspace exhausted");
        w.nmax = w.kmax + batch; w.zmax = w.kmax + 4 * (size_t)batch; w.wmax = w.kmax + 5 * (size_t)batch;
        w.pmax = w.kmax + 6 * (size_t)batch;
        w.Wp.KS = 4 * ((G2 + 63) / 64); w.Wp.JT = 2 * ((N + 63) / 64); w.Wp.count = batch;
        w.Wp.st = (long long)w.Wp.JT * w.Wp.KS * 256;
        w.Wp.data = a.get<uint4>((size_t)batch * w.Wp.st);
        w.Wp.bmax = w.wmax;
        JSTSP_REQUIRE(w.Wp.data, JSTSP_E_NOMEM, "proposed_algorithm: workspace exhausted");
        if (nB == 1 && hgemm_pair_shape(N, G2, batch)) {
            w.Kp.KS = 4 * ((M + 63) / 64); w.Kp.JT = 2; w.Kp.count = batch;
            w.Kp.st = (long long)w.Kp.JT * w.Kp.KS * 256;
            w.Kp.data = a.get<uint4>((size_t)batch * w.Kp.st);
            JSTSP_REQUIRE(w.Kp.data, JSTSP_E_NOMEM, "proposed_algorithm: workspace exhausted");
        }
    }
    w.h2g = use_hgemm(Gr, G2, G2);
    if (w.h2g && !w.pmax) {
        w.pmax = a.get<uint32_t>(2 * (size_t)batch);
        JSTSP_REQUIRE(w.pmax, JSTSP_E_NOMEM, "proposed_algorithm: workspace exhausted");
    }
    return 0;
}

}

using namespace jstsp;

static bool tune_host_pipeline()
{
    load_tuning();
    return tune().host_pipeline != 0;
}

static int proposed_impl(jstsp_ctx *ctx, int N, int M, int Gr, int G2, int batch,
                         const jstsp_c32 *subY_, const float *Omega_,
                         const jstsp_c32 *A_, long long strideA, const jstsp_c32 *B_,
                         long long strideB, int Imax, const double *tau_Y,
                         const double *tau_S, const double *rho, int type,
                         const int32_t *indx_S_, jstsp_c32 *S_out, jstsp_c32 *Y_out,
                         double *ce_out, int memspace, bool allow_fused, std::vector<int> *overflowed, PendingSolve *defer = nullptr)
{
    JSTSP_REQUIRE(ctx, JSTSP_E_NULL, "ctx is NULL");
    JSTSP_REQUIRE(subY_ && Omega_ && A_ && B_ && tau_Y && tau_S && rho && S_out, JSTSP_E_NULL,
                  "proposed_algorithm: NULL array argument");
    JSTSP_REQUIRE(N > 0 && M > 0 && Gr > 0 && G2 > 0 && batch > 0 && Imax >= 0, JSTSP_E_SHAPE,
                  "proposed_algorithm: bad shape N=%d M=%d Gr=%d G2=%d batch=%d Imax=%d", N, M, Gr, G2, batch,
                  Imax);
    JSTSP_REQUIRE(memspace == JSTSP_HOST || memspace == JSTSP_DEVICE, JSTSP_E_ARG, "bad memspace %d",
                  memspace);
    JSTSP_REQUIRE(type == JSTSP_TYPE_APPROXIMATE || type == JSTSP_TYPE_STD, JSTSP_E_ARG, "bad type %d", type);
    JSTSP_REQUIRE(std::min(N, M) <= 2048, JSTSP_E_UNSUPPORTED,
                  "proposed_algorithm: min(N, M) = %d > 2048 (order of the SVT's Gram eigenproblem)",
                  std::min(N, M));
    JSTSP_REQUIRE(strideA == 0 || strideA >= (long long)N * Gr, JSTSP_E_SHAPE, "strideA too small");
    JSTSP_REQUIRE(strideB == 0 || strideB >= (long long)G2 * M, JSTSP_E_SHAPE, "strideB too small");
    const bool approx = type == JSTSP_TYPE_APPROXIMATE;
    JSTSP_REQUIRE(approx || (N >= Gr && M >= G2), JSTSP_E_UNSUPPORTED,
                  "proposed_algorithm 'std': K2 = kron(B.', A) must have full column rank (N >= Gr, M >= G2); the "
                  "under-determined U\\(L\\k) of the reference returns a basic, not least-squares, solution");
    JSTSP_ENTER(ctx);

    const bool angles = indx_S_ != nullptr;
    const bool want_ce = ce_out != nullptr;
    const size_t nm = (size_t)N * M, g = (size_t)Gr * G2, ng = (size_t)N * G2;
    const int nA = strideA ? batch : 1, nB = strideB ? batch : 1;
    const size_t szA = strideA ? (size_t)strideA * (batch - 1) + (size_t)N * Gr : (size_t)N * Gr;
    const size_t szB = strideB ? (size_t)strideB * (batch - 1) + (size_t)G2 * M : (size_t)G2 * M;

    size_t need = proposed_bytes(N, M, Gr, G2, batch, nA, nB, angles, want_ce, std::max(Imax, 1));
    if (!approx)
        need += (pinv_fits(N, Gr) ? rnd256((size_t)nA * Gr * N * sizeof(float2))
                                  : rnd256((size_t)nA * Gr * Gr * sizeof(float2)) + hinv_bytes(Gr, nA)) +
                (pinv_fits(G2, M) ? rnd256((size_t)nB * M * G2 * sizeof(float2))
                                  : rnd256((size_t)nB * G2 * G2 * sizeof(float2)) + hinv_bytes(G2, nB));
    const Tuning &tn = tune();
    const int ftiles = (M % 32 == 0) ? M / 32 : 0;
    const int fparts = tn.fused_parts > 0 ? tn.fused_parts : (ftiles % 4 == 0 ? 4 : (ftiles % 2 == 0 ? 2 : 1));
    const bool want_fused = allow_fused && tn.fused != 0 && approx && Imax > 1 && fused_shape_ok(N, M, G2, fparts);
    if (want_fused) need += fused_bytes(M, G2, nB, batch, fparts);
    need += 1024;
    if (approx)
        need += rnd256((size_t)nA * Gr * Gr * sizeof(float2)) + 2 * rnd256((size_t)nB * (G2 / 2 + 1) * G2 * sizeof(float2));
    const bool host_compact = memspace == JSTSP_HOST && tn.host_compact != 0 && tn.toeplitz != 0 && nB > 1 && G2 >= 32 &&
                              strideB == (long long)G2 * M && (szB * sizeof(float2) >= ((size_t)64 << 20) || tn.host_compact >= 2) &&
                              (long long)G2 * M < (1ll << 31);
    const size_t compact_elems = host_compact ? host_toeplitz_compact_elems(G2, M, nB) : 0;
    if (memspace == JSTSP_HOST) {
        need += rnd256(batch * nm * sizeof(float2)) + rnd256(batch * nm * sizeof(float)) +
                rnd256(szA * sizeof(float2)) + rnd256(szB * sizeof(float2));
        if (angles) need += rnd256(batch * g * sizeof(int32_t));
        need += rnd256(compact_elems * sizeof(float2));
    }
    JSTSP_TRY(ctx->arena.reserve(need));
    ctx->arena.reset();

    const float2 *subY, *A, *B;
    const float *Omega;
    const int32_t *indx_S = nullptr;
    JSTSP_TRY(stage_in(ctx, reinterpret_cast<const float2 *>(subY_), batch * nm, memspace, &subY));
    JSTSP_TRY(stage_in(ctx, Omega_, batch * nm, memspace, &Omega));
    JSTSP_TRY(stage_in(ctx, reinterpret_cast<const float2 *>(A_), szA, memspace, &A));
    int known_gt = ctx->dict_block_hint;
    ctx->dict_block_hint = 0;
    if (host_compact) {
        float2 *Bd = ctx->arena.get<float2>(szB), *Cd = ctx->arena.get<float2>(compact_elems);
        JSTSP_REQUIRE(Bd && Cd, JSTSP_E_NOMEM, "workspace exhausted while staging an input");
        JSTSP_TRY(host_toeplitz_stage(ctx, reinterpret_cast<const float2 *>(B_), G2, M, nB, Bd, Cd, compact_elems, &known_gt));
        if (!known_gt) JSTSP_HIP(hipMemcpyAsync(Bd, B_, szB * sizeof(float2), hipMemcpyHostToDevice, ctx->stream));
        B = Bd;
    } else
    JSTSP_TRY(stage_in(ctx, reinterpret_cast<const float2 *>(B_), szB, memspace, &B));
    if (angles) JSTSP_TRY(stage_in(ctx, indx_S_, batch * g, memspace, &indx_S));
    if (memspace == JSTSP_DEVICE)
        JSTSP_REQUIRE(((uintptr_t)subY % 16 == 0) && ((uintptr_t)Omega % 8 == 0), JSTSP_E_ARG,
                      "device arrays must be 16-byte aligned");

    ProposedWS w;
    JSTSP_TRY(proposed_alloc(ctx->arena, w, N, M, Gr, G2, batch, nA, nB, angles, want_ce, std::max(Imax, 1)));

    {
        std::vector<TrialParams> hp(batch);
        for (int t = 0; t < batch; ++t) hp[t] = make_trial_params(rho[t], tau_Y[t], tau_S[t]);
        JSTSP_TRY(upload(ctx, w.prm, hp.data(), batch * sizeof(TrialParams)));
    }

    hipStream_t st = ctx->stream;
    JSTSP_HIP(hipMemsetAsync(w.X, 0, batch * nm * sizeof(float2), st));
    JSTSP_HIP(hipMemsetAsync(w.V1, 0, batch * nm * sizeof(float2), st));
    JSTSP_HIP(hipMemsetAsync(w.V2, 0, batch * nm * sizeof(float2), st));
    JSTSP_HIP(hipMemsetAsync(w.C, 0, batch * nm * sizeof(float2), st));
    JSTSP_HIP(hipMemsetAsync(w.Xs, 0, batch * nm * sizeof(float2), st));
    JSTSP_HIP(hipMemsetAsync(w.Y, 0, batch * nm * sizeof(float2), st));
    JSTSP_HIP(hipMemsetAsync(w.V, 0, batch * g * sizeof(float2), st));
    JSTSP_HIP(hipMemsetAsync(w.S, 0, batch * g * sizeof(float2), st));
    JSTSP_HIP(hipMemsetAsync(w.ce, 0, (size_t)batch * 3 * std::max(Imax, 1) * sizeof(double), st));
    JSTSP_TRY(launch_inv_d(ctx, (long long)nm, batch, Omega, 2.f, w.prm, w.invD));
    const bool omega_direct = ((uintptr_t)Omega % 16 == 0) && (nm % 4 == 0);
    if (angles) JSTSP_TRY(launch_rank_from_index(ctx, (int)g, batch, indx_S, w.rank));

    const Mat Am{A, strideA, N}, Bm{B, strideB, G2};
    const int toep_env = tn.toeplitz;
    int toep_gt = 0;
    bool toep_probed = false;
    const Mat GAm{w.GA, strideA ? (long long)Gr * Gr : 0, Gr}, GBm{w.GB, strideB ? (long long)G2 * G2 : 0, G2};
    float2 *GAlo = nullptr;
    if (approx) {
        GAlo = ctx->arena.get<float2>((size_t)nA * Gr * Gr);
        JSTSP_REQUIRE(GAlo, JSTSP_E_NOMEM, "proposed_algorithm: workspace exhausted (Gram refinement)");
        JSTSP_TRY(gram_f64(ctx, 'L', A, strideA, N, Gr, nA, w.GA, (long long)Gr * Gr, GAlo));
    } else
    JSTSP_TRY(gemm(ctx, 'C', 'N', Gr, Gr, N, nA, Am, Am, w.GA, (long long)Gr * Gr, Gr));
    if (toep_env != 0 && known_gt && strideB) {
        toep_gt = known_gt;
        toep_probed = true;
    } else
    if (toep_env != 0 && (long long)G2 * M < (1ll << 31) && approx) {
        JSTSP_TRY(fused_probe_toeplitz(ctx, ctx->arena, B, strideB, G2, M, nB, &toep_gt));
        toep_probed = true;
    }
    if (w.h2) {
        JSTSP_TRY(hgemm_pack(ctx, w.Bc, ctx->arena, B, strideB, G2, 1, 1, M, G2, nB, (long long)G2 * M));
    }
    if (approx) {
        if (toep_gt && toep_env >= 2 && M >= G2 / toep_gt) {
            float2 *G0 = ctx->arena.get<float2>((size_t)nB * toep_gt * G2), *G0lo = ctx->arena.get<float2>((size_t)nB * toep_gt * G2);
            JSTSP_REQUIRE(G0 && G0lo, JSTSP_E_NOMEM, "workspace exhausted (G_B block row)");
            GemmDesc dg = make_gemm('N', 'C', toep_gt, G2, M, nB, Bm, Bm, G0, (long long)toep_gt * G2, toep_gt);
            dg.force_m64 = 1; dg.C_lo = G0lo;
            JSTSP_TRY(launch_cgemm(ctx, dg, GEMM_MISC));
            JSTSP_TRY(toeplitz_gram_assemble(ctx, B, strideB, G2, M, toep_gt, nB, G0, G0lo, w.GB, nullptr));
            ctx->last_dict_block = toep_gt;
        } else {
            GemmDesc dg = make_gemm('N', 'C', G2, G2, M, nB, Bm, Bm, w.GB, (long long)G2 * G2, G2);
            dg.force_m64 = 1; dg.herm_upper = 1;
            JSTSP_TRY(launch_cgemm(ctx, dg, GEMM_MISC));
            JSTSP_TRY(hermitian_fill_lower(ctx, w.GB, (long long)G2 * G2, G2, nB));
        }
    } else if (w.h2) {
        {
            HGemmDesc hb{B, strideB, G2, w.Bc.bmax, w.Bc.data, w.Bc.st, w.Bc.bmax, 1, w.Bc.KS, w.Bc.JT, w.GB,
                         (long long)G2 * G2, G2, G2, G2, M, nB, EPI_NONE, nullptr, nullptr, nullptr};
            hb.herm_upper = 1;
            JSTSP_TRY(launch_hgemm(ctx, hb, nullptr));
            JSTSP_TRY(hermitian_fill_lower(ctx, w.GB, (long long)G2 * G2, G2, nB));
        }
    } else
    JSTSP_TRY(gemm(ctx, 'N', 'C', G2, G2, M, nB, Bm, Bm, w.GB, (long long)G2 * G2, G2));

    if (w.h2g && approx)
        JSTSP_TRY(hgemm_pack(ctx, w.GBp, ctx->arena, w.GB, strideB ? (long long)G2 * G2 : 0, 1, G2, 0, G2, G2, nB,
                             (long long)G2 * G2));
    float2 *PA = nullptr, *PB = nullptr;
    if (!approx) {
        JSTSP_TRY(diag_reset(ctx));
        if (pinv_fits(N, Gr)) {
            PA = ctx->arena.get<float2>((size_t)nA * Gr * N);
            JSTSP_REQUIRE(PA, JSTSP_E_NOMEM, "proposed_algorithm 'std': workspace exhausted");
            JSTSP_TRY(launch_pinv(ctx, N, Gr, nA, A, strideA, N, PA, (long long)Gr * N, Gr));
        }
        if (pinv_fits(G2, M)) {
            PB = ctx->arena.get<float2>((size_t)nB * M * G2);
            JSTSP_REQUIRE(PB, JSTSP_E_NOMEM, "proposed_algorithm 'std': workspace exhausted");
            JSTSP_TRY(launch_pinv(ctx, G2, M, nB, B, strideB, G2, PB, (long long)M * G2, M));
        }
        float2 *GAi = PA ? nullptr : ctx->arena.get<float2>((size_t)nA * Gr * Gr);
        float2 *GBi = PB ? nullptr : ctx->arena.get<float2>((size_t)nB * G2 * G2);
        JSTSP_REQUIRE((PA || GAi) && (PB || GBi), JSTSP_E_NOMEM, "proposed_algorithm 'std': workspace exhausted");
        const size_t mark = ctx->arena.off;
        if (!PA) {
            JSTSP_TRY(hermitian_inverse(ctx, Gr, nA, w.GA, GAi));
            ctx->arena.off = mark;
            JSTSP_HIP(hipMemcpyAsync(w.GA, GAi, (size_t)nA * Gr * Gr * sizeof(float2), hipMemcpyDeviceToDevice, st));
        }
        if (!PB) {
            JSTSP_TRY(hermitian_inverse(ctx, G2, nB, w.GB, GBi));
            ctx->arena.off = mark;
            JSTSP_HIP(hipMemcpyAsync(w.GB, GBi, (size_t)nB * G2 * G2 * sizeof(float2), hipMemcpyDeviceToDevice, st));
        }
    }
    const long long snm = (long long)nm, sg = (long long)g, sng = (long long)ng;
    constexpr int rv_refresh = 4;
    auto refresh_at = [](int it) -> bool { return it % rv_refresh == 0; };
    const bool overlap = tn.overlap >= 0 ? tn.overlap != 0 : want_fused;
    uint32_t *const kmax0 = w.kmax;
    JSTSP_TRY(ensure_side_streams(ctx));
    hipStream_t sm = ctx->stream, s1 = overlap ? ctx->side[0] : sm, s2 = overlap ? ctx->side[1] : sm;
    hipEvent_t ev_x = ctx->ev[0], ev_svt = ctx->ev[1], ev_gxv = ctx->ev[2], ev_c = ctx->ev[3], ev_gv2 = ctx->ev[4],
               ev_ce = ctx->ev[5], ev_lxv = ctx->ev[6];
    if (Imax > 0) {
        JSTSP_TRY(launch_form_z(ctx, snm, batch, w.X, w.V1, w.prm, w.Zb));
        JSTSP_TRY(svt_prepare(ctx, w.gz, w.Zb, w.prm, nullptr, true));
    }
    const bool fz = w.gz.left;
    const bool hmax = w.h2 && fz && N <= 64;
    const bool zfly = hmax && want_ce && gram3_nsplit(N, M, G2, want_ce) > 0 && w.gz.nsplit == w.gn.nsplit;
    float2 *Zbuf[2] = {w.Zb, w.Zb2};
    const bool fusedp = want_fused && hmax && (want_ce ? zfly : true);
    const bool fusedy = fusedp;
    FusedWS fw;
    if (fusedp) {
        if (toep_env != 0 && !toep_probed) JSTSP_TRY(fused_probe_toeplitz(ctx, ctx->arena, B, strideB, G2, M, nB, &toep_gt));
        ctx->last_dict_block = toep_gt;
        JSTSP_TRY(fused_alloc(ctx->arena, fw, M, G2, nB, batch, fparts, toep_gt, toep_env >= 2 && fusedy));
        JSTSP_TRY(fused_pack_b(ctx, fw, B, strideB, G2, M, nB, w.Bc.bmax));
        JSTSP_HIP(hipMemsetAsync(fw.ovf, 0, (size_t)batch * sizeof(uint32_t), sm));
    }
    const int fused_kback = tn.fused_kback;
    bool passed = false;
    hipEvent_t ev_q1 = ctx->ev[7], ev_v = ctx->ev[8], ev_rv = ctx->ev[9];
    const bool rv_fused1 = fusedp && tn.grad_fused != 0 && grad_fused_shape(N, Gr, G2);
    const bool rv_early_ok = rv_fused1 && zfly && w.h2g && overlap;
    bool rv_early = false;
    if (want_ce) JSTSP_TRY(lanczos_warm_reset(ctx, w.gn));
    for (int it = 0; it < Imax; ++it) {
        if (want_ce) w.gn.lz.call = it;
        float2 *Zc = fz ? Zbuf[it & 1] : w.Zb, *Zn = fz ? Zbuf[(it + 1) & 1] : w.Zb;
        if (w.h2) {
            const size_t boff = (size_t)(it & 1) * 8 * (size_t)batch;
            w.kmax = kmax0 + boff; w.nmax = w.kmax + batch; w.zmax = w.kmax + 4 * (size_t)batch;
            w.wmax = w.kmax + 5 * (size_t)batch; w.pmax = w.kmax + 6 * (size_t)batch;
            if (!passed) JSTSP_HIP(hipMemsetAsync(w.kmax, 0, 8 * (size_t)batch * sizeof(uint32_t), sm));
        } else if (w.h2g) JSTSP_HIP(hipMemsetAsync(w.pmax, 0, 2 * (size_t)batch * sizeof(uint32_t), sm));
        int apply_no = 0;
        bool next_zeroed = false;
        if (it > 0) JSTSP_HIP(hipStreamWaitEvent(sm, ev_svt, 0));
        if (it > 0 && want_ce) JSTSP_HIP(hipStreamWaitEvent(sm, ev_gxv, 0));
        if (passed) {
        } else if (fz) {
            JSTSP_TRY(launch_eye_minus(ctx, N, batch, w.gz.Q, w.gz.Q));
            GemmDesc dq = make_gemm('N', 'N', N, M, N, batch, Mat{w.gz.Q, (long long)N * N, N}, Mat{Zc, snm, N}, w.Y, snm, N);
            dq.epi = EPI_UPDATE_X; dq.prm = w.prm;
            dq.e_rw0 = w.V1; dq.e_w1 = w.X; dq.e_w2 = w.ZK;
            dq.e_r0 = w.V2; dq.e_r2 = w.Xs; dq.e_r3 = subY; dq.e_f0 = w.invD;
            dq.e_w3 = (it + 1 < Imax && (!zfly || fusedy)) ? Zn : nullptr;
            if (zfly && it > 0) { dq.B = w.X; dq.B2 = w.V1; }
            dq.epi_store_c = (it + 1 == Imax);
            if (w.h2) {
                dq.amax_out = w.kmax;
                if (N <= 64) { dq.amax_x = w.nmax; dq.amax_v1 = w.nmax + batch; dq.amax_z = w.zmax; }
            }
            JSTSP_TRY(launch_cgemm(ctx, dq, GEMM_MISC));
        } else {
            JSTSP_TRY(svt_apply(ctx, w.gz, Zc, w.Y));
            JSTSP_TRY(launch_update_x(ctx, snm, batch, w.X, w.V1, w.V2, w.C, w.Xs, w.Y, subY, w.invD, w.prm, w.ZK));
        }
        JSTSP_HIP(hipEventRecord(ev_x, sm));
        auto issue_s1 = [&](int stage) -> int {
            if (stage != 2) JSTSP_HIP(hipStreamWaitEvent(s1, ev_x, 0));
            StreamScope sc(ctx, s1);
            if (stage != 2 && !fz) JSTSP_TRY(launch_form_z(ctx, snm, batch, w.X, w.V1, w.prm, Zn));
            if (zfly) {
              if (stage != 2) {
                if (fusedp && it > 0) JSTSP_HIP(hipStreamWaitEvent(s1, ev_lxv, 0));
                JSTSP_TRY(launch_hgram3(ctx, w.X, w.V1, snm, N, M, batch, w.gz.nsplit, w.nmax, w.nmax + batch, w.zmax,
                                        w.prm, w.gz.Gpart, w.gn.Gpart, w.gn.Gpart + (size_t)batch * N * N * w.gn.nsplit));
                JSTSP_HIP(hipEventRecord(ev_gxv, s1));
                if (fusedp) {
                    JSTSP_HIP(hipStreamWaitEvent(s2, ev_gxv, 0));
                    StreamScope sc2(ctx, s2);
                    JSTSP_TRY(lmax_from_partials_range(ctx, w.gn, 0, 2 * batch, w.lam, true));
                    JSTSP_HIP(hipEventRecord(ev_lxv, s2));
                }
              }
              if (stage == 1) return 0;
                JSTSP_TRY(svt_prepare(ctx, w.gz, w.X, w.prm, nullptr, true, w.zmax, nullptr, true));
                if (fusedy) JSTSP_TRY(fused_pack_wq(ctx, fw, w.gz.Q, batch));
            } else {
                JSTSP_TRY(svt_prepare(ctx, w.gz, Zn, w.prm, nullptr, true, hmax ? w.zmax : nullptr));
                if (fusedy) JSTSP_TRY(fused_pack_wq(ctx, fw, w.gz.Q, batch));
            }
            JSTSP_HIP(hipEventRecord(ev_svt, s1));
            return 0;
        };
        const bool svt_split = passed && fusedp && zfly && it + 1 < Imax;
        if (it + 1 < Imax) JSTSP_TRY(issue_s1(svt_split ? 1 : 0));
        if (want_ce && !(zfly && it + 1 < Imax)) {
            JSTSP_HIP(hipStreamWaitEvent(s2, ev_x, 0));
            StreamScope sc(ctx, s2);
            JSTSP_TRY(gram_partials_range(ctx, w.gn, w.X, snm, 0, 2 * batch, hmax ? w.nmax : nullptr, nullptr, nullptr, true));
            JSTSP_HIP(hipEventRecord(ev_gxv, s2));
        }
        if (passed) {
            JSTSP_TRY(fused_reduce(ctx, fw, G2, M, batch, w.Tc));
        } else if (PB) {
            JSTSP_TRY(gemm(ctx, 'N', 'N', N, G2, M, batch, Mat{w.ZK, snm, N}, Mat{PB, strideB ? (long long)M * G2 : 0, M},
                           w.Tc, sng, N, 1.f, nullptr, 0, 0, 0.f, GEMM_CORRELATE));
        } else if (w.h2) {
            if (!fz) JSTSP_TRY(hgemm_absmax(ctx, w.ZK, snm, snm, batch, w.kmax));
            HGemmDesc hc{w.ZK, snm, N, w.kmax, w.Bc.data, strideB ? w.Bc.st : 0, w.Bc.bmax, strideB ? 1 : 0, w.Bc.KS,
                         w.Bc.JT, w.Tc, sng, N, N, G2, M, batch, EPI_NONE, nullptr, nullptr, nullptr};
            if (w.Kp.data && !strideB && w.Kp.KS == w.Bc.KS) {
                w.Kp.bmax = w.kmax;
                JSTSP_TRY(hgemm_repack(ctx, w.Kp, w.ZK, snm, N, 1, 0, M, N, w.kmax));
                hc.Ap = w.Kp.data; hc.sApt = w.Kp.st; hc.aKS = w.Kp.KS;
            }
            JSTSP_TRY(launch_hgemm(ctx, hc, "correlate"));
        } else
        JSTSP_TRY(gemm(ctx, 'N', 'C', N, G2, M, batch, Mat{w.ZK, snm, N}, Bm, w.Tc, sng, N, 1.f, nullptr, 0, 0,
                       0.f, GEMM_CORRELATE));
        const long long cnt_ll = std::min<long long>(10 + 5ll * (it + 1), (long long)g);
        const Mat GAl{GAlo, strideA ? (long long)Gr * Gr : 0, Gr};
        auto second_factor = [&](float2 *out, uint32_t *pm, bool exact) -> int {
            if (exact || !w.h2g) {
                GemmDesc dr = make_gemm('N', 'N', Gr, G2, G2, batch, Mat{w.P1, sg, Gr}, GBm, out, sg, Gr);
                dr.force_m64 = exact ? 1 : 0;
                return launch_cgemm(ctx, dr, GEMM_MISC);
            }
            HGemmDesc hg{w.P1, sg, Gr, pm, w.GBp.data, strideB ? w.GBp.st : 0, w.GBp.bmax, strideB ? 1 : 0,
                         w.GBp.KS, w.GBp.JT, out, sg, Gr, Gr, G2, G2, batch, EPI_NONE, nullptr, nullptr, nullptr};
            return launch_hgemm(ctx, hg, nullptr);
        };
        auto apply_R = [&](const float2 *Xin, float2 *out, bool exact) -> int {
            uint32_t *pm = w.pmax ? w.pmax + (size_t)(apply_no++ & 1) * batch : nullptr;
            if (exact && rv_fused1) {
                JSTSP_TRY(launch_grad_refresh_p1(ctx, Xin, w.GA, GAlo, strideA ? (long long)Gr * Gr : 0, w.P1, G2, batch));
                return second_factor(out, pm, exact);
            }
            if (exact) JSTSP_TRY(gemm(ctx, 'N', 'N', Gr, G2, Gr, batch, GAl, Mat{Xin, sg, Gr}, w.P1, sg, Gr));
            GemmDesc dp = make_gemm('N', 'N', Gr, G2, Gr, batch, GAm, Mat{Xin, sg, Gr}, w.P1, sg, Gr, 1.f, exact ? w.P1 : nullptr, sg,
                                    Gr, exact ? 1.f : 0.f);
            dp.amax_out = w.h2g ? pm : nullptr;
            JSTSP_TRY(launch_cgemm(ctx, dp, GEMM_MISC));
            return second_factor(out, pm, exact);
        };
        if (approx) {
            const bool refreshed = refresh_at(it);
            if (refreshed && rv_early) {
                JSTSP_HIP(hipStreamWaitEvent(sm, ev_rv, 0));
                rv_early = false;
            } else if (refreshed) JSTSP_TRY(apply_R(w.V, w.RV, true));
            if (svt_split && tn.grad_fused != 0 && w.h2g && grad_fused_shape(N, Gr, G2)) {
                uint32_t *pm = w.pmax + (size_t)(apply_no++ & 1) * batch;
                JSTSP_TRY(launch_grad_res_p1(ctx, A, strideA, w.Tc, w.RV, w.Res, w.GA, strideA ? (long long)Gr * Gr : 0, w.P1, pm,
                                             G2, batch));
                JSTSP_TRY(second_factor(w.RRes, pm, false));
            } else {
            GemmDesc dres = make_gemm('C', 'N', Gr, G2, N, batch, Am, Mat{w.Tc, sng, N}, w.Res, sg, Gr, 1.f, w.RV, sg, Gr, -1.f);
            JSTSP_TRY(launch_cgemm(ctx, dres, GEMM_MISC));
            JSTSP_TRY(apply_R(w.Res, w.RRes, false));
            }
            if (svt_split) {
                JSTSP_HIP(hipEventRecord(ev_q1, sm));
                JSTSP_HIP(hipStreamWaitEvent(s1, ev_q1, 0));
                JSTSP_TRY(issue_s1(2));
            }
            const bool early_next = rv_early_ok && it + 1 < Imax && refresh_at(it + 1);
            uint32_t *const nx_zero = (fusedp && tn.grad_fused != 0 && it + 1 < Imax) ? kmax0 + (size_t)((it + 1) & 1) * 8 * (size_t)batch : nullptr;
            if (nx_zero && it > 0 && want_ce) JSTSP_HIP(hipStreamWaitEvent(sm, ev_gv2, 0));
            next_zeroed = nx_zero != nullptr;
            JSTSP_TRY(launch_step_v(ctx, (int)g, batch, w.Res, w.RRes, w.V, w.S, w.rank, (int)cnt_ll, w.prm, w.ce,
                                    Imax, it, early_next ? nullptr : w.RV, svt_split, nx_zero));
            if (early_next) {
                JSTSP_HIP(hipEventRecord(ev_v, sm));
                JSTSP_HIP(hipStreamWaitEvent(s2, ev_v, 0));
                StreamScope sc(ctx, s2);
                JSTSP_TRY(launch_grad_refresh_p1(ctx, w.V, w.GA, GAlo, strideA ? (long long)Gr * Gr : 0, w.P1, G2, batch));
                JSTSP_TRY(second_factor(w.RV, nullptr, true));
                JSTSP_HIP(hipEventRecord(ev_rv, s2));
                rv_early = true;
            }
        } else {
            float2 *left = PB ? w.V : w.P1;
            if (PA)
                JSTSP_TRY(gemm(ctx, 'N', 'N', Gr, G2, N, batch, Mat{PA, strideA ? (long long)Gr * N : 0, Gr},
                               Mat{w.Tc, sng, N}, left, sg, Gr));
            else {
                JSTSP_TRY(gemm(ctx, 'C', 'N', Gr, G2, N, batch, Am, Mat{w.Tc, sng, N}, w.Res, sg, Gr));
                JSTSP_TRY(gemm(ctx, 'N', 'N', Gr, G2, Gr, batch, GAm, Mat{w.Res, sg, Gr}, left, sg, Gr));
            }
            if (!PB) JSTSP_TRY(gemm(ctx, 'N', 'N', Gr, G2, G2, batch, Mat{w.P1, sg, Gr}, GBm, w.V, sg, Gr));
            JSTSP_TRY(launch_soft(ctx, (int)g, batch, w.V, w.S, w.rank, (int)cnt_ll, w.prm));
        }
        if (fusedp && !want_ce && it + 1 == Imax) break;
        if (w.h2) {
            GemmDesc dw = make_gemm('N', 'N', N, G2, Gr, batch, Am, Mat{w.S, sg, Gr}, w.W, sng, N);
            dw.amax_out = w.wmax;
            JSTSP_TRY(launch_cgemm(ctx, dw, GEMM_MISC));
        } else
        JSTSP_TRY(gemm(ctx, 'N', 'N', N, G2, Gr, batch, Am, Mat{w.S, sg, Gr}, w.W, sng, N));
        if (it > 0 && want_ce) JSTSP_HIP(hipStreamWaitEvent(sm, ev_gv2, 0));
        passed = false;
        if (fusedp && it + 1 < Imax) {
            uint32_t *nx = kmax0 + (size_t)((it + 1) & 1) * 8 * (size_t)batch;
            if (!next_zeroed) JSTSP_HIP(hipMemsetAsync(nx, 0, 8 * (size_t)batch * sizeof(uint32_t), sm));
            JSTSP_TRY(fused_pack_as(ctx, fw, w.W, sng, G2, M, batch, w.wmax));
            JSTSP_HIP(hipStreamWaitEvent(sm, ev_svt, 0));
            FusedDesc fd{fw.Bf, strideB ? fw.sBf : 0, w.Bc.bmax, strideB ? 1 : 0, fw.ASp, fw.sAS, w.wmax, w.kmax,
                         w.X, w.V1, w.V2, subY, w.Y, omega_direct ? Omega : w.invD, snm, w.prm, fw.Ppart,
                         nx, nx + batch, nx + 2 * (size_t)batch, nx + 4 * (size_t)batch, w.nmax + 2 * (size_t)batch, fw.ovf,
                         M, G2, batch, fparts,
                         fusedy ? fw.Wqp : nullptr, Zbuf[(it + 1) & 1], w.zmax,
                         (fw.v2 && zfly) ? nullptr : Zbuf[it & 1],
                         (fusedy && it + 2 == Imax) ? w.Y : nullptr, fused_kback,
                         fw.Ec, strideB ? fw.sEc : 0, fw.gt ? 31 - __builtin_clz((unsigned)fw.gt) : 0, fw.ecols, fw.ehalo,
                         fw.v2, fw.XsD, fw.Kf, omega_direct ? 1 : 0};
            JSTSP_TRY(launch_fused_pass(ctx, fd));
            passed = true;
        } else
        if (w.h2) {
            JSTSP_TRY(hgemm_repack(ctx, w.Wp, w.W, sng, N, 1, 0, G2, N, w.wmax));
            if (!w.Bs.data)
                JSTSP_TRY(hgemm_pack(ctx, w.Bs, ctx->arena, B, strideB, 1, G2, 0, G2, M, nB, (long long)G2 * M, w.Bc.bmax));
            HGemmDesc hs{w.W, sng, N, w.wmax, w.Bs.data, strideB ? w.Bs.st : 0, w.Bs.bmax, strideB ? 1 : 0, w.Bs.KS,
                         w.Bs.JT, w.Xs, snm, N, N, M, G2, batch, fz ? EPI_UPDATE_C : EPI_NONE, w.prm, w.X, w.V2,
                         hmax ? w.nmax + 2 * (size_t)batch : nullptr, w.Wp.data, w.Wp.st, w.Wp.KS};
            JSTSP_TRY(launch_hgemm(ctx, hs, "synthesize"));
            if (!fz) JSTSP_TRY(launch_update_c(ctx, snm, batch, w.X, w.Xs, w.V2, w.C, w.prm));
        } else if (fz) {
            GemmDesc ds = make_gemm('N', 'N', N, M, G2, batch, Mat{w.W, sng, N}, Bm, w.Xs, snm, N);
            ds.epi = EPI_UPDATE_C; ds.prm = w.prm;
            ds.e_r0 = w.X; ds.e_rw0 = w.V2;
            JSTSP_TRY(launch_cgemm(ctx, ds, GEMM_SYNTH));
        } else {
            JSTSP_TRY(gemm(ctx, 'N', 'N', N, M, G2, batch, Mat{w.W, sng, N}, Bm, w.Xs, snm, N, 1.f, nullptr, 0, 0,
                           0.f, GEMM_SYNTH));
            JSTSP_TRY(launch_update_c(ctx, snm, batch, w.X, w.Xs, w.V2, w.C, w.prm));
        }
        if (want_ce) {
            JSTSP_HIP(hipEventRecord(ev_c, sm));
            JSTSP_HIP(hipStreamWaitEvent(s2, ev_c, 0));
            if (zfly) JSTSP_HIP(hipStreamWaitEvent(s2, ev_gxv, 0));
            StreamScope sc(ctx, s2);
            JSTSP_TRY(gram_partials_range(ctx, w.gn, w.X, snm, 2 * batch, batch, hmax ? w.nmax : nullptr, nullptr, nullptr, true));
            JSTSP_HIP(hipEventRecord(ev_gv2, s2));
            if (fusedp && zfly && it + 1 < Imax) JSTSP_TRY(lmax_from_partials_range(ctx, w.gn, 2 * batch, batch, w.lam, true));
            else JSTSP_TRY(lmax_from_partials(ctx, w.gn, w.lam, true));
            JSTSP_TRY(launch_ce_ratio(ctx, batch, w.lam + batch, w.lam + 2 * batch, w.lam, w.ce, Imax, it));
            JSTSP_HIP(hipEventRecord(ev_ce, s2));
        }
    }
    if (want_ce && Imax > 0) JSTSP_HIP(hipStreamWaitEvent(sm, ev_ce, 0));
    if (defer) {
        defer->active = true; defer->fused = fusedp; defer->want_ce = want_ce && Imax > 0; defer->batch = batch; defer->g = g; defer->nm = nm;
        defer->Imax = Imax; defer->dS = w.S; defer->dY = w.Y; defer->dce = w.ce; defer->ovf = fusedp ? fw.ovf : nullptr;
        return 0;
    }

    JSTSP_TRY(stage_out(ctx, reinterpret_cast<float2 *>(S_out), w.S, batch * g, memspace));
    JSTSP_TRY(stage_out(ctx, reinterpret_cast<float2 *>(Y_out), w.Y, batch * nm, memspace));
    if (want_ce && Imax > 0) JSTSP_TRY(stage_out(ctx, ce_out, w.ce, (size_t)batch * 3 * Imax, memspace));
    if (fusedp && overflowed) {
        std::vector<uint32_t> flags(batch);
        JSTSP_HIP(hipMemcpyAsync(flags.data(), fw.ovf, (size_t)batch * sizeof(uint32_t), hipMemcpyDeviceToHost, st));
        JSTSP_HIP(hipStreamSynchronize(st));
        for (int t = 0; t < batch; ++t)
            if (flags[t]) overflowed->push_back(t);
    }
    if (memspace == JSTSP_HOST) {
        JSTSP_HIP(hipStreamSynchronize(st));
        if (!approx) JSTSP_TRY(diag_check_host(ctx, "proposed_algorithm 'std'"));
    }
    return 0;
}

static int resolve_overflowed(jstsp_ctx *ctx, const std::vector<int> &ovf, int N, int M, int Gr, int G2, const jstsp_c32 *subY,
                              const float *Omega, const jstsp_c32 *A, long long strideA, const jstsp_c32 *B, long long strideB,
                              int Imax, const double *tau_Y, const double *tau_S, const double *rho, int type,
                              const int32_t *indx_S, jstsp_c32 *S_out, jstsp_c32 *Y_out, double *ce_out, int memspace, int *count)
{
    const size_t nm = (size_t)N * M, g = (size_t)Gr * G2;
    for (size_t i = 0; i < ovf.size();) {
        size_t j = i + 1;
        while (j < ovf.size() && ovf[j] == ovf[j - 1] + 1) ++j;
        const int t0 = ovf[i], cnt = (int)(j - i);
        JSTSP_TRY(proposed_impl(ctx, N, M, Gr, G2, cnt, subY + t0 * nm, Omega + t0 * nm, A + (size_t)t0 * strideA, strideA,
                                B + (size_t)t0 * strideB, strideB, Imax, tau_Y + t0, tau_S + t0, rho + t0, type,
                                indx_S ? indx_S + t0 * g : nullptr, S_out + t0 * g, Y_out ? Y_out + t0 * nm : nullptr,
                                ce_out ? ce_out + (size_t)t0 * 3 * Imax : nullptr, memspace, false, nullptr));
        *count += cnt;
        i = j;
    }
    return 0;
}

static int proposed_finish(jstsp_ctx *ctx, const PendingSolve &p, jstsp_c32 *S_out, jstsp_c32 *Y_out, double *ce_out, std::vector<int> *ovf)
{
    JSTSP_ENTER(ctx);
    JSTSP_TRY(stage_out(ctx, reinterpret_cast<float2 *>(S_out), p.dS, p.batch * p.g, JSTSP_HOST));
    JSTSP_TRY(stage_out(ctx, reinterpret_cast<float2 *>(Y_out), p.dY, p.batch * p.nm, JSTSP_HOST));
    if (p.want_ce) JSTSP_TRY(stage_out(ctx, ce_out, p.dce, (size_t)p.batch * 3 * p.Imax, JSTSP_HOST));
    std::vector<uint32_t> flags(p.ovf ? p.batch : 0);
    if (p.ovf) JSTSP_HIP(hipMemcpyAsync(flags.data(), p.ovf, (size_t)p.batch * sizeof(uint32_t), hipMemcpyDeviceToHost, ctx->stream));
    JSTSP_HIP(hipStreamSynchronize(ctx->stream));
    for (int t = 0; t < (int)flags.size(); ++t)
        if (flags[t]) ovf->push_back(t);
    return 0;
}

// ... 178 lines not shown
```

jstsp19_amd/csrc/solver_common.h:

```cpp
#pragma once
#include "common.h"
#include <vector>

namespace jstsp {

struct Mat {
    const float2 *p; long long st; int ld;
};

int gemm(jstsp_ctx *ctx, char opA, char opB, int m, int n, int k, int batch, Mat A, Mat B, float2 *C,
         long long sCt, int ldc, float alpha = 1.f, const float2 *D = nullptr, long long sDt = 0,
         int ldd = 0, float beta = 0.f, int tag = GEMM_MISC, int splitk = 1, long long sCsplit = 0);

int gram_f64(jstsp_ctx *ctx, char side, const float2 *X, long long sXt, int rows, int cols, int count, float2 *G, long long sGt,
             float2 *Glo = nullptr);

bool grad_head_shape_ok(int N, int Gr, int G2);
int launch_grad_head(jstsp_ctx *ctx, int G2, int batch, const float2 *P, long long sPt, long long sPp, int parts, const float2 *Kf,
                     const float2 *Bdl, long long sBdl, const float2 *A, long long sA, const float2 *GA, long long sGA,
                     const float2 *RV, float2 *Tc, float2 *Res, float2 *P1, uint32_t *pmax);

GemmDesc make_gemm(char opA, char opB, int m, int n, int k, int batch, Mat A, Mat B, float2 *C, long long sCt,
                   int ldc, float alpha = 1.f, const float2 *D = nullptr, long long sDt = 0, int ldd = 0,
                   float beta = 0.f, int splitk = 1, long long sCsplit = 0);
// ... 45 lines not shown
int ensure_diag(jstsp_ctx *ctx);
int diag_reset(jstsp_ctx *ctx);
int diag_check_host(jstsp_ctx *ctx, const char *what);

struct PendingSolve {
    bool active = false, fused = false, want_ce = false;
    int batch = 0;
    size_t g = 0, nm = 0;
    int Imax = 0;
    const float2 *dS = nullptr, *dY = nullptr;
    const double *dce = nullptr;
    const uint32_t *ovf = nullptr;
};
int proposed_enqueue_device(jstsp_ctx *ctx, int N, int M, int Gr, int G2, int batch, const jstsp_c32 *subY, const float *Omega,
                            const jstsp_c32 *A, long long strideA, const jstsp_c32 *B, long long strideB, int Imax,
                            const double *tau_Y, const double *tau_S, const double *rho, int type, const int32_t *indx_S,
                            bool want_ce, PendingSolve *out);
int proposed_pending_flags(jstsp_ctx *ctx, const PendingSolve &p, std::vector<int> *ovf);
int proposed_resolve_device(jstsp_ctx *ctx, int N, int M, int Gr, int G2, int batch, const jstsp_c32 *subY, const float *Omega,
                            const jstsp_c32 *A, long long strideA, const jstsp_c32 *B, long long strideB, int Imax,
                            const double *tau_Y, const double *tau_S, const double *rho, int type, const int32_t *indx_S,
                            jstsp_c32 *S_dev, jstsp_c32 *Y_dev, double *ce_dev);

int upload(jstsp_ctx *ctx, void *dst, const void *src, size_t bytes);

template <class T> int stage_in(jstsp_ctx *ctx, const T *src, size_t n, int memspace, const T **out)
{
    if (memspace == JSTSP_DEVICE) { *out = src; return 0; }
    T *d = ctx->arena.get<T>(n);
    JSTSP_REQUIRE(d, JSTSP_E_NOMEM, "workspace exhausted while staging an input");
    JSTSP_HIP(hipMemcpyAsync(d, src, n * sizeof(T), hipMemcpyHostToDevice, ctx->stream));
    *out = d;
    return 0;
}
template <class T> int stage_out(jstsp_ctx *ctx, T *dst, const T *dev, size_t n, int memspace)
{
    if (!dst) return 0;
    JSTSP_HIP(hipMemcpyAsync(dst, dev, n * sizeof(T),
                             memspace == JSTSP_DEVICE ? hipMemcpyDeviceToDevice : hipMemcpyDeviceToHost,
                             ctx->stream));
    return 0;
}
inline size_t rnd256(size_t b) { return (b + 255) & ~size_t(255); }

template <class T>
int host_toeplitz_stage(jstsp_ctx *ctx, const T *Bh, int G2, int M, int nB, float2 *Bdev, float2 *Cdev, size_t cdev_elems, int *gt_out);
size_t host_toeplitz_compact_elems(int G2, int M, int nB);

struct FusedWS {
    uint4 *Bf = nullptr; long long sBf = 0;
    uint4 *ASp = nullptr; long long sAS = 0;
    float2 *Ppart = nullptr;
    uint32_t *ovf = nullptr;
    uint4 *Wqp = nullptr;
    int parts = 0;
    uint4 *Ec = nullptr; long long sEc = 0;
    int gt = 0, ecols = 0, ehalo = 0;
    int v2 = 0;
    const float2 *Bsrc = nullptr; long long sBsrc = 0;
    float2 *Bdl = nullptr; long long sBdl = 0;
    float2 *XsD = nullptr, *Kf = nullptr;
};
struct FusedDesc {
    const uint4 *Bf; long long sBf;
    const uint32_t *bmax; int sbmax;
    const uint4 *ASp; long long sAS;
    const uint32_t *wmax;
    const uint32_t *kmax_prev;
    float2 *X, *V1, *V2;
    const float2 *subY, *Y; const float *invD;
    long long snm;
    const TrialParams *prm;
    float2 *Ppart;
    uint32_t *kmax_out, *xmax, *v1max, *zmax, *v2max, *ovf;
    int M, G2, batch, parts;
    const uint4 *Wqp; const float2 *Zin; const uint32_t *zmax_in; float2 *Zout, *Yout;
    int kback;
    const uint4 *Ec; long long sEc; int gsh, ecols, ehalo;
    int v2; const float2 *XsD; float2 *Kf;
    int inv_is_omega;
};
bool fused_shape_ok(int N, int M, int G2, int parts);
size_t fused_bytes(int M, int G2, int nB, int batch, int parts);
int fused_probe_toeplitz(jstsp_ctx *ctx, Arena &ar, const float2 *B, long long sBt, int G2, int M, int nB, int *gt);
int toeplitz_gram_assemble(jstsp_ctx *ctx, const float2 *B, long long sBt, int G2, int M, int gt, int nB, const float2 *G0,
                           const float2 *G0lo, float2 *G, float2 *Glo);
int fused_alloc(Arena &ar, FusedWS &f, int M, int G2, int nB, int batch, int parts, int gt, int v2);
int fused_pack_b(jstsp_ctx *ctx, FusedWS &f, const float2 *B, long long sBt, int G2, int M, int nB, const uint32_t *bmax);
int fused_pack_as(jstsp_ctx *ctx, const FusedWS &f, const float2 *W, long long sWt, int G2, int M, int batch, const uint32_t *wmax);
int launch_fused_pass(jstsp_ctx *ctx, const FusedDesc &d);
int fused_reduce(jstsp_ctx *ctx, const FusedWS &f, int G2, int M, int batch, float2 *Tc);
int fused_pack_wq(jstsp_ctx *ctx, const FusedWS &f, const float2 *Q, int batch);

bool grad_fused_shape(int N, int Gr, int G2);
int launch_grad_res_p1(jstsp_ctx *ctx, const float2 *A, long long sAt, const float2 *Tc, const float2 *RV, float2 *Res,
                       const float2 *GA, long long sGAt, float2 *P1, uint32_t *pmax, int G2, int batch);
int launch_grad_refresh_p1(jstsp_ctx *ctx, const float2 *V, const float2 *GA, const float2 *GAlo, long long sGAt, float2 *P1, int G2,
                           int batch);

}
```

Baseline: 842.0 channel-estimates/s.

## Read fp32 dictionary directly in hgemm and fold absmax into Toeplitz probe

Adds a direct-B mode to the split-f16 hgemm kernels: the dictionary B is loaded as fp32 and converted to hi/lo f16 in the staging store, so the correlate and synthesize GEMMs no longer need separately packed copies of B. The Toeplitz probe and verify kernels are merged into one synchronized launch pair, and the verify kernel also computes per-trial B absmax, which removes a separate absmax pass. Packing of B now happens lazily only when the fused or packed path actually needs it. The cost is more per-tile conversion work and strided fp32 loads inside the GEMM. A new API entry for testing the dictionary product is also added.

```diff
diff --git a/include/jstsp.h b/include/jstsp.h
--- a/include/jstsp.h
+++ b/include/jstsp.h
@@ -80,6 +80,10 @@
 int jstsp_lambda_max_sequence_c32(jstsp_ctx *ctx, int n, int batch, int steps, const jstsp_c32 *G, float *lam, int memspace);
 
 int jstsp_last_dictionary_block(jstsp_ctx *ctx, int *gt);
+
+int jstsp_dictionary_product_c32(jstsp_ctx *ctx, int orient, int direct, int probe_bmax, int N, int M, int G2, int batch,
+                                 const jstsp_c32 *a, const jstsp_c32 *B, long long strideB, jstsp_c32 *out,
+                                 const jstsp_c32 *X, jstsp_c32 *V2, unsigned int *bmax_out, int *from_probe, int *gt_out);
 
 int jstsp_ls_c32(jstsp_ctx *ctx, int N, int M, int Gr, int G2, int batch, const jstsp_c32 *Y,
                  const jstsp_c32 *A, long long strideA, const jstsp_c32 *B, long long strideB,
diff --git a/jstsp19_amd/_lib.py b/jstsp19_amd/_lib.py
--- a/jstsp19_amd/_lib.py
+++ b/jstsp19_amd/_lib.py
@@ -62,6 +62,8 @@
     "jstsp_last_fused_fallbacks": (c_int, [c_void_p, c_ip]),
     "jstsp_last_lanczos_mismatches": (c_int, [c_void_p, c_ip]),
     "jstsp_last_dictionary_block": (c_int, [c_void_p, c_ip]),
+    "jstsp_dictionary_product_c32": (c_int, [c_void_p, c_int, c_int, c_int, c_int, c_int, c_int, c_int, c_void_p, c_void_p, c_ll,
+                                             c_void_p, c_void_p, c_void_p, c_void_p, c_ip, c_ip]),
     "jstsp_svt_c32": (c_int, [c_void_p, c_int, c_int, c_int, c_void_p, c_dp, c_void_p, c_int]),
     "jstsp_omp_c32": (c_int, [c_void_p, c_int, c_int, c_int, c_void_p, c_ll, c_void_p, c_int, c_void_p,
                               c_void_p, c_void_p, c_int]),
diff --git a/jstsp19_amd/csrc/api_misc.hip b/jstsp19_amd/csrc/api_misc.hip
--- a/jstsp19_amd/csrc/api_misc.hip
+++ b/jstsp19_amd/csrc/api_misc.hip
@@ -686,3 +686,58 @@
     if (memspace == JSTSP_HOST) JSTSP_HIP(hipStreamSynchronize(ctx->stream));
     return 0;
 }
+
+extern "C" int jstsp_dictionary_product_c32(jstsp_ctx *ctx, int orient, int direct, int probe_bmax, int N, int M, int G2, int batch,
+                                            const jstsp_c32 *a_, const jstsp_c32 *B_, long long strideB, jstsp_c32 *out_,
+                                            const jstsp_c32 *X_, jstsp_c32 *V2_, unsigned int *bmax_out, int *from_probe, int *gt_out)
+{
+    JSTSP_TRY(check_common(ctx, JSTSP_DEVICE));
+    JSTSP_ENTER(ctx);
+    JSTSP_REQUIRE(a_ && B_ && out_ && (orient == 0 || (X_ && V2_)), JSTSP_E_NULL, "dictionary_product: NULL array argument");
+    JSTSP_REQUIRE((orient == 0 || orient == 1) && N > 0 && N <= 64 && M > 0 && G2 > 0 && batch > 0, JSTSP_E_SHAPE,
+                  "dictionary_product: bad shape");
+    JSTSP_REQUIRE(strideB == 0 || strideB >= (long long)G2 * M, JSTSP_E_SHAPE, "strideB too small");
+    const int nB = strideB ? batch : 1;
+    const long long nm = (long long)N * M, ng = (long long)N * G2;
+    const int Kd = orient ? G2 : M, J = orient ? M : G2;
+    const size_t need = hgemm_pack_bytes(Kd, J, nB) + hgemm_pack_bytes(G2, N, batch) + 4 * rnd256((size_t)(batch + nB) * sizeof(uint32_t)) +
+                        rnd256((size_t)batch * sizeof(TrialParams)) + 4096;
+    JSTSP_TRY(ctx->arena.reserve(need));
+    ctx->arena.reset();
+    const float2 *a = reinterpret_cast<const float2 *>(a_), *B = reinterpret_cast<const float2 *>(B_);
+    uint32_t *bmax = ctx->arena.get<uint32_t>(nB), *amax = ctx->arena.get<uint32_t>(batch);
+    JSTSP_REQUIRE(bmax && amax, JSTSP_E_NOMEM, "dictionary_product: workspace exhausted");
+    bool done = false;
+    int gt = 0;
+    if (probe_bmax && (long long)G2 * M < (1ll << 31))
+        JSTSP_TRY(fused_probe_toeplitz(ctx, ctx->arena, B, strideB, G2, M, nB, &gt, bmax, &done));
+    if (from_probe) *from_probe = done ? 1 : 0;
+    if (gt_out) *gt_out = gt;
+    if (!done) JSTSP_TRY(hgemm_absmax(ctx, B, (long long)G2 * M, strideB, nB, bmax));
+    if (bmax_out) JSTSP_HIP(hipMemcpyAsync(bmax_out, bmax, (size_t)nB * sizeof(uint32_t), hipMemcpyDeviceToDevice, ctx->stream));
+    JSTSP_TRY(hgemm_absmax(ctx, a, orient ? ng : nm, orient ? ng : nm, batch, amax));
+    HGemmDesc hd{a, orient ? ng : nm, N, amax, nullptr, 0, bmax, strideB ? 1 : 0, 4 * ((Kd + 63) / 64), 4 * ((J + 127) / 128),
+                 reinterpret_cast<float2 *>(out_), orient ? nm : ng, N, N, J, Kd, batch, EPI_NONE, nullptr, nullptr, nullptr};
+    if (orient) {
+        std::vector<TrialParams> hp(batch, make_trial_params(1.0, 1.0, 1.0));
+        TrialParams *prm = ctx->arena.get<TrialParams>(batch);
+        HPack wp;
+        wp.KS = 4 * ((G2 + 63) / 64); wp.JT = 2 * ((N + 63) / 64); wp.count = batch; wp.st = (long long)wp.JT * wp.KS * 256;
+        wp.data = ctx->arena.get<uint4>((size_t)batch * wp.st);
+        JSTSP_REQUIRE(prm && wp.data, JSTSP_E_NOMEM, "dictionary_product: workspace exhausted");
+        JSTSP_TRY(upload(ctx, prm, hp.data(), batch * sizeof(TrialParams)));
+        JSTSP_TRY(hgemm_repack(ctx, wp, a, ng, N, 1, 0, G2, N, amax));
+        hd.epi = EPI_UPDATE_C; hd.prm = prm; hd.e_r0 = reinterpret_cast<const float2 *>(X_); hd.e_rw0 = reinterpret_cast<float2 *>(V2_);
+        hd.Ap = wp.data; hd.sApt = wp.st; hd.aKS = wp.KS;
+    }
+    if (direct) {
+        hd.Bd = B; hd.sBdt = strideB; hd.ldb = G2; hd.bdir = orient ? HGEMM_B_SYNTH : HGEMM_B_CORRELATE;
+    } else {
+        HPack pk;
+        if (orient) JSTSP_TRY(hgemm_pack(ctx, pk, ctx->arena, B, strideB, 1, G2, 0, G2, M, nB, (long long)G2 * M, bmax));
+        else JSTSP_TRY(hgemm_pack(ctx, pk, ctx->arena, B, strideB, G2, 1, 1, M, G2, nB, (long long)G2 * M, bmax));
+        hd.Bp = pk.data; hd.sPt = strideB ? pk.st : 0;
+    }
+    JSTSP_TRY(launch_hgemm(ctx, hd, nullptr));
+    return 0;
+}
diff --git a/jstsp19_amd/csrc/common.h b/jstsp19_amd/csrc/common.h
--- a/jstsp19_amd/csrc/common.h
+++ b/jstsp19_amd/csrc/common.h
@@ -258,7 +258,10 @@
     const uint4 *Ap; long long sApt; int aKS;
     int herm_upper;
     int map_tb, map_tt;
-};
+    const float2 *Bd; long long sBdt; int ldb; int bdir;
+};
+enum { HGEMM_B_PACKED = 0, HGEMM_B_CORRELATE = 1, HGEMM_B_SYNTH = 2 };
+bool hgemm_direct_ok(const HGemmDesc &d);
 int hermitian_fill_lower(jstsp_ctx *ctx, float2 *G, long long sGt, int n, int count);
 int launch_hgram(jstsp_ctx *ctx, const float2 *Z, long long sZt, int rows, int cols, int count, int nsplit,
                  const uint32_t *amax, float2 *Gpart, const float2 *Z2 = nullptr,
diff --git a/jstsp19_amd/csrc/fused.hip b/jstsp19_amd/csrc/fused.hip
--- a/jstsp19_amd/csrc/fused.hip
+++ b/jstsp19_amd/csrc/fused.hip
@@ -102,18 +102,26 @@
     if ((threadIdx.x & 63) == 0 && (bad & ~__atomic_load_n(mism, __ATOMIC_RELAXED))) atomicOr(mism, bad);
 }
 
-__global__ __launch_bounds__(256) void toeplitz_verify_kernel(const float2 *B, long long sBt, int G2, int M, int c, uint32_t *mism)
+__global__ __launch_bounds__(256) void toeplitz_verify_kernel(const float2 *B, long long sBt, int G2, int M, uint32_t cand, uint32_t *mism,
+                                                              uint32_t *bmax)
 {
     const uint32_t q = blockIdx.x * 256u + threadIdx.x;
     const uint32_t qpc = (uint32_t)G2 >> 2;
+    const uint32_t surv = cand & ~__atomic_load_n(mism - 1, __ATOMIC_RELAXED);
+    const int c = surv ? __builtin_ctz(surv) : -1;
     uint32_t bad = 0;
+    float mx = 0.f;
     if (q < qpc * (uint32_t)M) {
         const int m = (int)(q / qpc), g = 4 * (int)(q - (uint32_t)m * qpc);
-        const int gt = 16 << c, ld = g >> (4 + c);
+        const int gt = c >= 0 ? 16 << c : 0, ld = c >= 0 ? g >> (4 + c) : 0;
+        const uint4 *b = reinterpret_cast<const uint4 *>(reinterpret_cast<const uint2 *>(B) + (long long)blockIdx.y * sBt);
+        const uint32_t e = (uint32_t)g + (uint32_t)G2 * (uint32_t)m;
+        const uint4 x0 = b[e >> 1], x1 = b[(e >> 1) + 1];
+        mx = fmaxf(fmaxf(fmaxf(fabsf(__uint_as_float(x0.x)), fabsf(__uint_as_float(x0.y))),
+                         fmaxf(fabsf(__uint_as_float(x0.z)), fabsf(__uint_as_float(x0.w)))),
+                   fmaxf(fmaxf(fabsf(__uint_as_float(x1.x)), fabsf(__uint_as_float(x1.y))),
+                         fmaxf(fabsf(__uint_as_float(x1.z)), fabsf(__uint_as_float(x1.w)))));
         if (ld >= 1 && m >= ld) {
-            const uint4 *b = reinterpret_cast<const uint4 *>(reinterpret_cast<const uint2 *>(B) + (long long)blockIdx.y * sBt);
-            const uint32_t e = (uint32_t)g + (uint32_t)G2 * (uint32_t)m;
-            const uint4 x0 = b[e >> 1], x1 = b[(e >> 1) + 1];
             const uint32_t f = e - (uint32_t)gt - (uint32_t)G2;
             const uint4 y0 = b[f >> 1], y1 = b[(f >> 1) + 1];
             if (x0.x != y0.x || x0.y != y0.y || x0.z != y0.z || x0.w != y0.w || x1.x != y1.x || x1.y != y1.y || x1.z != y1.z ||
@@ -122,8 +130,13 @@
         }
     }
 #pragma unroll
-    for (int o = 32; o > 0; o >>= 1) bad |= __shfl_xor(bad, o);
+    for (int o = 32; o > 0; o >>= 1) { bad |= __shfl_xor(bad, o); mx = fmaxf(mx, __shfl_xor(mx, o)); }
     if ((threadIdx.x & 63) == 0 && (bad & ~__atomic_load_n(mism, __ATOMIC_RELAXED))) atomicOr(mism, bad);
+    __shared__ float sm[4];
+    if ((threadIdx.x & 63) == 0) sm[threadIdx.x >> 6] = mx;
+    __syncthreads();
+    if (threadIdx.x == 0)
+        atomicMax(&bmax[blockIdx.y], __float_as_uint(fmaxf(fmaxf(sm[0], sm[1]), fmaxf(sm[2], sm[3]))));
 }
 
 __global__ __launch_bounds__(256) void pack_e_kernel(const float2 *B, long long sBt, int G2, int M, int gt, int ecols, int ehalo,
@@ -966,23 +979,40 @@
            rnd256((size_t)nB * G2 * 8 * sizeof(float2)) + 512;
 }
 
-int fused_probe_toeplitz(jstsp_ctx *ctx, Arena &ar, const float2 *B, long long sBt, int G2, int M, int nB, int *gt)
+int fused_probe_toeplitz(jstsp_ctx *ctx, Arena &ar, const float2 *B, long long sBt, int G2, int M, int nB, int *gt, uint32_t *bmax,
+                         bool *bmax_done)
 {
     *gt = 0;
-    uint32_t *flag = ar.get<uint32_t>(1);
+    if (bmax_done) *bmax_done = false;
+    uint32_t *flag = ar.get<uint32_t>(2);
     JSTSP_REQUIRE(flag, JSTSP_E_NOMEM, "fused pass: workspace exhausted");
     JSTSP_REQUIRE((long long)G2 * M < (1ll << 31), JSTSP_E_UNSUPPORTED, "fused pass: dictionary too large");
     uint32_t cand = 0;
     for (int c = 0; c < 5; ++c)
         if (G2 % (16 << c) == 0 && 2 * (16 << c) <= G2) cand |= 1u << c;
     const unsigned nblk = (unsigned)(((long long)G2 * M + 255) / 256);
+    if (nB > 1 && sBt % 2 == 0 && cand && G2 % 4 == 0) {
+        uint32_t bad[2] = {~0u, ~0u};
+        uint32_t *bm = bmax;
+        if (!bm) { bm = ar.get<uint32_t>(nB); JSTSP_REQUIRE(bm, JSTSP_E_NOMEM, "fused pass: workspace exhausted"); }
+        JSTSP_HIP(hipMemsetAsync(flag, 0, 2 * sizeof(uint32_t), ctx->stream));
+        JSTSP_HIP(hipMemsetAsync(bm, 0, (size_t)nB * sizeof(uint32_t), ctx->stream));
+        hipLaunchKernelGGL(toeplitz_probe_kernel, dim3(nblk, 1), dim3(256), 0, ctx->stream, B, sBt, G2, M, cand, flag);
+        JSTSP_HIP(hipGetLastError());
+        hipLaunchKernelGGL(toeplitz_verify_kernel, dim3((nblk + 3) / 4, nB), dim3(256), 0, ctx->stream, B, sBt, G2, M, cand, flag + 1, bm);
+        JSTSP_HIP(hipGetLastError());
+        JSTSP_HIP(hipMemcpyAsync(bad, flag, 2 * sizeof(uint32_t), hipMemcpyDeviceToHost, ctx->stream));
+        JSTSP_HIP(hipStreamSynchronize(ctx->stream));
+        cand &= ~bad[0];
+        cand &= cand ? (~cand + 1u) : 0u;
+        cand &= ~bad[1];
+        if (cand) *gt = 16 << (31 - __builtin_clz(cand));
+        if (bmax && bmax_done) *bmax_done = true;
+        return 0;
+    }
     for (int step = 0; step < (nB > 1 ? 2 : 1) && cand; ++step) {
         JSTSP_HIP(hipMemsetAsync(flag, 0, sizeof(uint32_t), ctx->stream));
-        if (step && sBt % 2 == 0)
-            hipLaunchKernelGGL(toeplitz_verify_kernel, dim3((nblk + 3) / 4, nB), dim3(256), 0, ctx->stream, B, sBt, G2, M,
-                               31 - __builtin_clz(cand), flag);
-        else
-            hipLaunchKernelGGL(toeplitz_probe_kernel, dim3(nblk, step ? nB : 1), dim3(256), 0, ctx->stream, B, sBt, G2, M, cand, flag);
+        hipLaunchKernelGGL(toeplitz_probe_kernel, dim3(nblk, step ? nB : 1), dim3(256), 0, ctx->stream, B, sBt, G2, M, cand, flag);
         JSTSP_HIP(hipGetLastError());
         uint32_t bad = ~0u;
         JSTSP_HIP(hipMemcpyAsync(&bad, flag, sizeof(uint32_t), hipMemcpyDeviceToHost, ctx->stream));
diff --git a/jstsp19_amd/csrc/hgemm.hip b/jstsp19_amd/csrc/hgemm.hip
--- a/jstsp19_amd/csrc/hgemm.hip
+++ b/jstsp19_amd/csrc/hgemm.hip
@@ -6,6 +6,8 @@
 typedef _Float16 half8 __attribute__((ext_vector_type(8)));
 typedef float f32x16 __attribute__((ext_vector_type(16)));
 typedef unsigned int u32x4 __attribute__((ext_vector_type(4)));
+typedef float f32x2 __attribute__((ext_vector_type(2)));
+typedef float f32x4 __attribute__((ext_vector_type(4)));
 
 namespace {
 
@@ -103,9 +105,10 @@
     return t < d.batch && tile < tiles;
 }
 
-template <int EPI, bool APACK, int WJ, bool EVEN = false>
+template <int EPI, bool APACK, int WJ, bool EVEN = false, bool BDIR = false>
 __global__ __launch_bounds__(128 * WJ, WJ == 2 ? 2 : 2) void hgemm_kernel(HGemmDesc d, int tiles_i, int tiles_j)
 {
+    static_assert(!BDIR || !APACK, "the direct b operand comes with an fp32 a operand");
     constexpr int STG = 1024 + 512 * WJ;
     constexpr int NA = (WJ == 2) ? 8 : 4;
     __shared__ uint4 smem[2 * STG];
@@ -135,21 +138,36 @@
     const int kfull = d.k / HBK;
 
     struct StgF { float2 a[NA]; uint4 b0, b1, b2, b3; };
+    struct StgD { float2 a[NA]; f32x2 b[8]; };
     struct StgP { u32x4 a0, a1, a2, a3; uint4 b0, b1, b2, b3; };
-    using Stg = typename std::conditional<APACK, StgP, StgF>::type;
+    using Stg = typename std::conditional<BDIR, StgD, typename std::conditional<APACK, StgP, StgF>::type>::type;
     const uint4 *pbw = pb + ((long long)(wave >> 1) * d.KS + (wave & 1)) * 256;
+    const int bj = j0 + (wave >> 1) * 32 + (lane & 31), bk0 = (wave & 1) * 16 + 8 * (lane >> 5);
+    const bool brow = bj < d.n;
+    const f32x2 *pbd = BDIR ? reinterpret_cast<const f32x2 *>(d.Bd + (long long)t * d.sBdt + (brow ? bj : 0)) : nullptr;
+    const float sb = ldexpf(1.f, eb);
     const uint4 *paw = APACK ? d.Ap + (long long)t * d.sApt + lane +
                                    ((long long)(ti * 2 + (wave >> 1)) * d.KS + (wave & 1)) * 256
                              : nullptr;
     const float sa_m = arow ? sa : 0.f;
     auto load = [&](int s_in, Stg &R) {
         const int s = EVEN ? (s_in < nst ? s_in : 0) : s_in;
+        if constexpr (BDIR) {
+#pragma unroll
+            for (int v = 0; v < 8; ++v) {
+                const int kk = s * HBK + bk0 + v;
+                const bool ok = brow && (EVEN || kk < d.k);
+                const f32x2 x = __builtin_nontemporal_load(pbd + (long long)((EVEN || kk < d.k) ? kk : 0) * d.ldb);
+                R.b[v] = ok ? x : f32x2{0.f, 0.f};
+            }
+        } else {
         const uint4 *g = pbw + (long long)(2 * s) * 256;
         const u32x4 *gn = reinterpret_cast<const u32x4 *>(g);
         const u32x4 x0 = __builtin_nontemporal_load(gn), x1 = __builtin_nontemporal_load(gn + 64),
                     x2 = __builtin_nontemporal_load(gn + 128), x3 = __builtin_nontemporal_load(gn + 192);
         R.b0 = make_uint4(x0.x, x0.y, x0.z, x0.w); R.b1 = make_uint4(x1.x, x1.y, x1.z, x1.w);
         R.b2 = make_uint4(x2.x, x2.y, x2.z, x2.w); R.b3 = make_uint4(x3.x, x3.y, x3.z, x3.w);
+        }
         if constexpr (APACK) {
             const u32x4 *ga = reinterpret_cast<const u32x4 *>(paw + (long long)(2 * s) * 256);
             R.a0 = ga[0]; R.a1 = ga[64]; R.a2 = ga[128]; R.a3 = ga[192];
@@ -171,7 +189,19 @@
     };
     auto store = [&](const Stg &R, uint4 *buf) {
         uint4 *o = buf + 1024 + wave * 256 + lane;
-        o[0] = R.b0; o[64] = R.b1; o[128] = R.b2; o[192] = R.b3;
+        if constexpr (BDIR) {
+            half8 rh, rl, ih, il;
+#pragma unroll
+            for (int v = 0; v < 8; ++v) {
+                _Float16 h, l;
+                split2(R.b[v].x * sb, h, l); rh[v] = h; rl[v] = l;
+                split2(R.b[v].y * -sb, h, l); ih[v] = h; il[v] = l;
+            }
+            o[0] = *reinterpret_cast<uint4 *>(&rh); o[64] = *reinterpret_cast<uint4 *>(&rl);
+            o[128] = *reinterpret_cast<uint4 *>(&ih); o[192] = *reinterpret_cast<uint4 *>(&il);
+        } else {
+            o[0] = R.b0; o[64] = R.b1; o[128] = R.b2; o[192] = R.b3;
+        }
         if constexpr (APACK) {
             u32x4 *q = reinterpret_cast<u32x4 *>(buf + wave * 256 + lane);
             q[0] = R.a0; q[64] = R.a1; q[128] = R.a2; q[192] = R.a3;
@@ -373,7 +403,7 @@
     }
 }
 
-template <int EPI, bool APACK, int NW, int PD>
+template <int EPI, bool APACK, int NW, int PD, bool BDIR = false>
 __global__ __launch_bounds__(64 * NW, NW == 4 ? 2 : 1) void hgemm2_kernel(HGemmDesc d, int tiles_j)
 {
     constexpr int NT = 64 * NW;
@@ -454,10 +484,28 @@
     const uint4 *pbw = d.Bp + (long long)t * d.sPt + ((long long)(tj * NW + wave) * d.KS) * 256 + lane;
     struct BStg { u32x4 q[8]; };
     const uint4 *pdummy = APACK ? d.Ap + (long long)t * d.sApt + lane : pbw;
+    const int bj = j0 + wave * 32 + (lane & 31);
+    const bool bcol = bj < d.n;
+    const f32x4 *pbd = BDIR ? reinterpret_cast<const f32x4 *>(d.Bd + (long long)t * d.sBdt + (long long)(bcol ? bj : 0) * d.ldb +
+                                                              8 * (lane >> 5))
+                            : nullptr;
+    const float sb = ldexpf(1.f, eb);
     auto load_b_half = [&](int s, int ks, BStg &R) {
+        if constexpr (BDIR) {
+            const int k0 = (2 * s + ks) * 16 + 8 * (lane >> 5);
+            const bool ok = s < nst && k0 < d.k;
+            const f32x4 *g = pbd + (ok ? (2 * s + ks) * 8 : 0);
+            const bool live = ok && bcol;
+#pragma unroll
+            for (int p = 0; p < 4; ++p) {
+                const f32x4 x = __builtin_nontemporal_load(g + p);
+                R.q[ks * 4 + p] = __builtin_bit_cast(u32x4, live ? x : f32x4{0.f, 0.f, 0.f, 0.f});
+            }
+        } else {
         const u32x4 *g = reinterpret_cast<const u32x4 *>(s < nst ? pbw + (long long)(2 * s + ks) * 256 : pdummy);
 #pragma unroll
         for (int p = 0; p < 4; ++p) R.q[ks * 4 + p] = __builtin_nontemporal_load(g + p * 64);
+        }
     };
 
     f32x16 re[2], im[2];
@@ -469,8 +517,20 @@
     auto nh8 = [](u32x4 u) { u.x ^= 0x80008000u; u.y ^= 0x80008000u; u.z ^= 0x80008000u; u.w ^= 0x80008000u;
                              return *reinterpret_cast<half8 *>(&u); };
     auto compute_half = [&](const uint4 *buf, int ks, const BStg &R) {
-        const half8 br_h = h8(R.q[ks * 4 + 0]), br_l = h8(R.q[ks * 4 + 1]), bi_h = h8(R.q[ks * 4 + 2]),
-                    bi_l = h8(R.q[ks * 4 + 3]);
+        half8 br_h, br_l, bi_h, bi_l;
+        if constexpr (BDIR) {
+#pragma unroll
+            for (int p = 0; p < 4; ++p) {
+                const f32x4 x = __builtin_bit_cast(f32x4, R.q[ks * 4 + p]);
+                _Float16 h, l;
+                split2(x.x * sb, h, l); br_h[2 * p] = h; br_l[2 * p] = l;
+                split2(x.y * sb, h, l); bi_h[2 * p] = h; bi_l[2 * p] = l;
+                split2(x.z * sb, h, l); br_h[2 * p + 1] = h; br_l[2 * p + 1] = l;
+                split2(x.w * sb, h, l); bi_h[2 * p + 1] = h; bi_l[2 * p + 1] = l;
+            }
+        } else {
+            br_h = h8(R.q[ks * 4 + 0]); br_l = h8(R.q[ks * 4 + 1]); bi_h = h8(R.q[ks * 4 + 2]); bi_l = h8(R.q[ks * 4 + 3]);
+        }
         const u32x4 *fa0 = reinterpret_cast<const u32x4 *>(buf + ((0 * 2 + ks) * 4) * 64 + lane);
         const u32x4 *fa1 = reinterpret_cast<const u32x4 *>(buf + ((1 * 2 + ks) * 4) * 64 + lane);
         const u32x4 u0r_h = fa0[0], u0r_l = fa0[64], u0i_h = fa0[128], u0i_l = fa0[192];
@@ -1184,9 +1244,26 @@
     return m == 64 && batch >= 2 && (long long)((batch + 1) / 2) * ((n + 127) / 128) >= 256;
 }
 
+bool hgemm_direct_ok(const HGemmDesc &d)
+{
+    if (!d.Bd || d.m <= 0 || d.n <= 0 || d.k <= 0) return false;
+    const bool pack_ok = d.JT * 32 >= ((d.n + 127) / 128) * 128 && d.KS == 4 * ((d.k + 63) / 64);
+    if (d.bdir == HGEMM_B_CORRELATE)
+        return !d.Ap && d.epi == EPI_NONE && !d.herm_upper && d.n >= 128 && pack_ok && d.ldb >= d.n;
+    if (d.bdir == HGEMM_B_SYNTH)
+        return d.Ap && d.aKS == d.KS && d.m <= 64 && pack_ok && d.epi == EPI_UPDATE_C && !d.herm_upper &&
+               !(d.sBdt == 0 && hgemm_pair_shape(d.m, d.n, d.batch)) && d.k >= 16 && (d.k % 8) == 0 && (d.ldb % 2) == 0 && (d.sBdt % 2) == 0 &&
+               (((uintptr_t)d.Bd) & 15) == 0 && d.ldb >= d.k;
+    return false;
+}
+
 int launch_hgemm(jstsp_ctx *ctx, const HGemmDesc &d_in, const char *prof_name)
 {
     HGemmDesc d = d_in;
+    if (d.bdir != HGEMM_B_PACKED) {
+        JSTSP_REQUIRE(hgemm_direct_ok(d), JSTSP_E_UNSUPPORTED, "hgemm: this product does not take an unpacked b operand");
+        d.Bp = nullptr; d.sPt = d.sBdt ? 1 : 0;
+    }
     JSTSP_REQUIRE(d.m > 0 && d.n > 0 && d.k > 0 && d.batch > 0, JSTSP_E_SHAPE, "hgemm: bad shape");
     JSTSP_REQUIRE(d.KS >= 2 * ((d.k + 31) / 32) && d.JT >= 2 * ((d.n + 63) / 64), JSTSP_E_ARG,
                   "hgemm: packed operand smaller than the product");
@@ -1222,7 +1299,9 @@
         const int tj2 = (d.n + 127) / 128;
         const long long grid2 = hgemm_grid(d, tj2, 64);
         if (prof_name) prof_begin(ctx, prof_name);
-        if (d.epi == EPI_UPDATE_C)
+        if (d.bdir == HGEMM_B_SYNTH)
+            hgemm2_kernel<EPI_UPDATE_C, true, 4, 2, true><<<(unsigned)grid2, 256, 0, ctx->stream>>>(d, tj2);
+        else if (d.epi == EPI_UPDATE_C)
             hgemm2_kernel<EPI_UPDATE_C, true, 4, 2><<<(unsigned)grid2, 256, 0, ctx->stream>>>(d, tj2);
         else
             hgemm2_kernel<EPI_NONE, true, 4, 2><<<(unsigned)grid2, 256, 0, ctx->stream>>>(d, tj2);
@@ -1241,7 +1320,10 @@
     }
     const long long grid = hgemm_grid(d, (long long)tiles_i * tiles_j, wide ? 32 : 64);
     if (prof_name) prof_begin(ctx, prof_name);
-    if (wide_even) {
+    if (d.bdir == HGEMM_B_CORRELATE) {
+        if (wide_even) hgemm_kernel<EPI_NONE, false, 4, true, true><<<(unsigned)grid, 512, 0, ctx->stream>>>(d, tiles_i, tiles_j);
+        else hgemm_kernel<EPI_NONE, false, 4, false, true><<<(unsigned)grid, 512, 0, ctx->stream>>>(d, tiles_i, tiles_j);
+    } else if (wide_even) {
         hgemm_kernel<EPI_NONE, false, 4, true><<<(unsigned)grid, 512, 0, ctx->stream>>>(d, tiles_i, tiles_j);
     } else if (wide) {
         hgemm_kernel<EPI_NONE, false, 4><<<(unsigned)grid, 512, 0, ctx->stream>>>(d, tiles_i, tiles_j);
diff --git a/jstsp19_amd/csrc/proposed.hip b/jstsp19_amd/csrc/proposed.hip
--- a/jstsp19_amd/csrc/proposed.hip
+++ b/jstsp19_amd/csrc/proposed.hip
@@ -170,7 +170,7 @@
     const int fparts = tn.fused_parts > 0 ? tn.fused_parts : (ftiles % 4 == 0 ? 4 : (ftiles % 2 == 0 ? 2 : 1));
     const bool want_fused = allow_fused && tn.fused != 0 && approx && Imax > 1 && fused_shape_ok(N, M, G2, fparts);
     if (want_fused) need += fused_bytes(M, G2, nB, batch, fparts);
-    need += 1024;
+    need += 1024 + 2 * rnd256((size_t)nB * sizeof(uint32_t));
     if (approx)
         need += rnd256((size_t)nA * Gr * Gr * sizeof(float2)) + 2 * rnd256((size_t)nB * (G2 / 2 + 1) * G2 * sizeof(float2));
     const bool host_compact = memspace == JSTSP_HOST && tn.host_compact != 0 && tn.toeplitz != 0 && nB > 1 && G2 >= 32 &&
@@ -242,17 +242,33 @@
         JSTSP_TRY(gram_f64(ctx, 'L', A, strideA, N, Gr, nA, w.GA, (long long)Gr * Gr, GAlo));
     } else
     JSTSP_TRY(gemm(ctx, 'C', 'N', Gr, Gr, N, nA, Am, Am, w.GA, (long long)Gr * Gr, Gr));
+    uint32_t *bmaxB = nullptr;
+    bool bmaxB_done = false;
+    if (w.h2) {
+        bmaxB = ctx->arena.get<uint32_t>(nB);
+        JSTSP_REQUIRE(bmaxB, JSTSP_E_NOMEM, "proposed_algorithm: workspace exhausted");
+    }
     if (toep_env != 0 && known_gt && strideB) {
         toep_gt = known_gt;
         toep_probed = true;
     } else
     if (toep_env != 0 && (long long)G2 * M < (1ll << 31) && approx) {
-        JSTSP_TRY(fused_probe_toeplitz(ctx, ctx->arena, B, strideB, G2, M, nB, &toep_gt));
+        JSTSP_TRY(fused_probe_toeplitz(ctx, ctx->arena, B, strideB, G2, M, nB, &toep_gt, bmaxB, &bmaxB_done));
         toep_probed = true;
     }
-    if (w.h2) {
-        JSTSP_TRY(hgemm_pack(ctx, w.Bc, ctx->arena, B, strideB, G2, 1, 1, M, G2, nB, (long long)G2 * M));
-    }
+    auto need_bmax = [&]() -> int {
+        if (!bmaxB_done) JSTSP_TRY(hgemm_absmax(ctx, B, (long long)G2 * M, strideB, nB, bmaxB));
+        bmaxB_done = true;
+        return 0;
+    };
+    const int KSc = 4 * ((M + 63) / 64), JTc = 4 * ((G2 + 127) / 128);
+    const int KSs = 4 * ((G2 + 63) / 64), JTs = 4 * ((M + 127) / 128);
+    auto pack_bc = [&]() -> int {
+        if (w.Bc.data) return 0;
+        JSTSP_TRY(need_bmax());
+        return hgemm_pack(ctx, w.Bc, ctx->arena, B, strideB, G2, 1, 1, M, G2, nB, (long long)G2 * M, bmaxB);
+    };
+    if (w.h2 && (!want_fused || tn.fused == 2)) JSTSP_TRY(pack_bc());
     if (approx) {
         if (toep_gt && toep_env >= 2 && M >= G2 / toep_gt) {
             float2 *G0 = ctx->arena.get<float2>((size_t)nB * toep_gt * G2), *G0lo = ctx->arena.get<float2>((size_t)nB * toep_gt * G2);
@@ -270,6 +286,7 @@
         }
     } else if (w.h2) {
         {
+            JSTSP_TRY(pack_bc());
             HGemmDesc hb{B, strideB, G2, w.Bc.bmax, w.Bc.data, w.Bc.st, w.Bc.bmax, 1, w.Bc.KS, w.Bc.JT, w.GB,
                          (long long)G2 * G2, G2, G2, G2, M, nB, EPI_NONE, nullptr, nullptr, nullptr};
             hb.herm_upper = 1;
@@ -329,12 +346,14 @@
     float2 *Zbuf[2] = {w.Zb, w.Zb2};
     const bool fusedp = want_fused && hmax && (want_ce ? zfly : true);
     const bool fusedy = fusedp;
+    const bool b_direct = fusedp && tn.fused != 2;
     FusedWS fw;
     if (fusedp) {
         if (toep_env != 0 && !toep_probed) JSTSP_TRY(fused_probe_toeplitz(ctx, ctx->arena, B, strideB, G2, M, nB, &toep_gt));
         ctx->last_dict_block = toep_gt;
         JSTSP_TRY(fused_alloc(ctx->arena, fw, M, G2, nB, batch, fparts, toep_gt, toep_env >= 2 && fusedy));
-        JSTSP_TRY(fused_pack_b(ctx, fw, B, strideB, G2, M, nB, w.Bc.bmax));
+        JSTSP_TRY(need_bmax());
+        JSTSP_TRY(fused_pack_b(ctx, fw, B, strideB, G2, M, nB, bmaxB));
         JSTSP_HIP(hipMemsetAsync(fw.ovf, 0, (size_t)batch * sizeof(uint32_t), sm));
     }
     const int fused_kback = tn.fused_kback;
@@ -419,9 +438,18 @@
                            w.Tc, sng, N, 1.f, nullptr, 0, 0, 0.f, GEMM_CORRELATE));
         } else if (w.h2) {
             if (!fz) JSTSP_TRY(hgemm_absmax(ctx, w.ZK, snm, snm, batch, w.kmax));
-            HGemmDesc hc{w.ZK, snm, N, w.kmax, w.Bc.data, strideB ? w.Bc.st : 0, w.Bc.bmax, strideB ? 1 : 0, w.Bc.KS,
-                         w.Bc.JT, w.Tc, sng, N, N, G2, M, batch, EPI_NONE, nullptr, nullptr, nullptr};
-            if (w.Kp.data && !strideB && w.Kp.KS == w.Bc.KS) {
+            HGemmDesc hc{w.ZK, snm, N, w.kmax, nullptr, 0, bmaxB, strideB ? 1 : 0, KSc,
+                         JTc, w.Tc, sng, N, N, G2, M, batch, EPI_NONE, nullptr, nullptr, nullptr};
+            const bool kpair = w.Kp.data && !strideB && w.Kp.KS == KSc;
+            if (b_direct && !kpair) {
+                hc.Bd = B; hc.sBdt = strideB; hc.ldb = G2; hc.bdir = HGEMM_B_CORRELATE;
+                if (!hgemm_direct_ok(hc)) { hc.Bd = nullptr; hc.bdir = HGEMM_B_PACKED; }
+            }
+            if (hc.bdir == HGEMM_B_PACKED) {
+                JSTSP_TRY(pack_bc());
+                hc.Bp = w.Bc.data; hc.sPt = strideB ? w.Bc.st : 0;
+            } else JSTSP_TRY(need_bmax());
+            if (kpair) {
                 w.Kp.bmax = w.kmax;
                 JSTSP_TRY(hgemm_repack(ctx, w.Kp, w.ZK, snm, N, 1, 0, M, N, w.kmax));
                 hc.Ap = w.Kp.data; hc.sApt = w.Kp.st; hc.aKS = w.Kp.KS;
@@ -517,7 +545,7 @@
             if (!next_zeroed) JSTSP_HIP(hipMemsetAsync(nx, 0, 8 * (size_t)batch * sizeof(uint32_t), sm));
             JSTSP_TRY(fused_pack_as(ctx, fw, w.W, sng, G2, M, batch, w.wmax));
             JSTSP_HIP(hipStreamWaitEvent(sm, ev_svt, 0));
-            FusedDesc fd{fw.Bf, strideB ? fw.sBf : 0, w.Bc.bmax, strideB ? 1 : 0, fw.ASp, fw.sAS, w.wmax, w.kmax,
+            FusedDesc fd{fw.Bf, strideB ? fw.sBf : 0, bmaxB, strideB ? 1 : 0, fw.ASp, fw.sAS, w.wmax, w.kmax,
                          w.X, w.V1, w.V2, subY, w.Y, omega_direct ? Omega : w.invD, snm, w.prm, fw.Ppart,
                          nx, nx + batch, nx + 2 * (size_t)batch, nx + 4 * (size_t)batch, w.nmax + 2 * (size_t)batch, fw.ovf,
                          M, G2, batch, fparts,
@@ -531,11 +559,19 @@
         } else
         if (w.h2) {
             JSTSP_TRY(hgemm_repack(ctx, w.Wp, w.W, sng, N, 1, 0, G2, N, w.wmax));
-            if (!w.Bs.data)
-                JSTSP_TRY(hgemm_pack(ctx, w.Bs, ctx->arena, B, strideB, 1, G2, 0, G2, M, nB, (long long)G2 * M, w.Bc.bmax));
-            HGemmDesc hs{w.W, sng, N, w.wmax, w.Bs.data, strideB ? w.Bs.st : 0, w.Bs.bmax, strideB ? 1 : 0, w.Bs.KS,
-                         w.Bs.JT, w.Xs, snm, N, N, M, G2, batch, fz ? EPI_UPDATE_C : EPI_NONE, w.prm, w.X, w.V2,
+            HGemmDesc hs{w.W, sng, N, w.wmax, nullptr, 0, bmaxB, strideB ? 1 : 0, KSs,
+                         JTs, w.Xs, snm, N, N, M, G2, batch, fz ? EPI_UPDATE_C : EPI_NONE, w.prm, w.X, w.V2,
                          hmax ? w.nmax + 2 * (size_t)batch : nullptr, w.Wp.data, w.Wp.st, w.Wp.KS};
+            if (b_direct) {
+                hs.Bd = B; hs.sBdt = strideB; hs.ldb = G2; hs.bdir = HGEMM_B_SYNTH;
+                if (!hgemm_direct_ok(hs)) { hs.Bd = nullptr; hs.bdir = HGEMM_B_PACKED; }
+            }
+            JSTSP_TRY(need_bmax());
+            if (hs.bdir == HGEMM_B_PACKED) {
+                if (!w.Bs.data)
+                    JSTSP_TRY(hgemm_pack(ctx, w.Bs, ctx->arena, B, strideB, 1, G2, 0, G2, M, nB, (long long)G2 * M, bmaxB));
+                hs.Bp = w.Bs.data; hs.sPt = strideB ? w.Bs.st : 0;
+            }
             JSTSP_TRY(launch_hgemm(ctx, hs, "synthesize"));
             if (!fz) JSTSP_TRY(launch_update_c(ctx, snm, batch, w.X, w.Xs, w.V2, w.C, w.prm));
         } else if (fz) {
diff --git a/jstsp19_amd/csrc/solver_common.h b/jstsp19_amd/csrc/solver_common.h
--- a/jstsp19_amd/csrc/solver_common.h
+++ b/jstsp19_amd/csrc/solver_common.h
@@ -151,7 +151,8 @@
 };
 bool fused_shape_ok(int N, int M, int G2, int parts);
 size_t fused_bytes(int M, int G2, int nB, int batch, int parts);
-int fused_probe_toeplitz(jstsp_ctx *ctx, Arena &ar, const float2 *B, long long sBt, int G2, int M, int nB, int *gt);
+int fused_probe_toeplitz(jstsp_ctx *ctx, Arena &ar, const float2 *B, long long sBt, int G2, int M, int nB, int *gt,
+                         uint32_t *bmax = nullptr, bool *bmax_done = nullptr);
 int toeplitz_gram_assemble(jstsp_ctx *ctx, const float2 *B, long long sBt, int G2, int M, int gt, int nB, const float2 *G0,
                            const float2 *G0lo, float2 *G, float2 *Glo);
 int fused_alloc(Arena &ar, FusedWS &f, int M, int G2, int nB, int batch, int parts, int gt, int v2);
```

Measured after the change: 845.6 channel-estimates/s (median of 6 runs). Within noise of the previous version (+0.4%).
